# gregspangenberg/shoulder

Measured on AMD Instinct MI355X. Metric: humerus meshes/s end-to-end (all 4 landmarks), higher is better.
Workload: dtype f64 geometry + bf16 UNet

## Files before the change

shoulder_amd/csrc/hull.hip:

```cpp
#include "sh_ctx.h"

#include "k_hullpre.h"
#include "k_hull.h"
#include "sh_hull.h"

using namespace sh;

static int alloc_hulld(sh_ctx* c) {
  const int B = c->B;
  int rc;
  ENS("hulld.fv", (size_t)B * HD_SLOTS * 3 * 4, 4);
  ENS("hulld.vis", (size_t)B * HD_KC * HD_VMAX * 4, 4);
  ENS("hulld.ev", (size_t)B * HD_KC * 3 * HD_VMAX * 2 * 4, 4);
  ENS("hulld.hor", (size_t)B * HD_KC * (HD_VMAX + 2) * 2 * 4, 4);
  ENS("hulld.newslot", (size_t)B * HD_SLOTS * 4, 4);
  ENS("hulld.freestack", (size_t)B * HD_SLOTS * 4, 4);
  ENS("hulld.tkeys", (size_t)B * HD_TBL * 8, 8);
  ENS("hulld.tvals", (size_t)B * HD_TBL * 4, 4);
  ENS("hulld.fail", (size_t)B * 4, 4);
  ENS("hulld.rounds", (size_t)B * 4, 4);
  ENS("hulld.skip", (size_t)B * 4, 4);
  if (c->skip_gen != c->batch_gen) {
    HIPCHK(c, hipMemsetAsync(c->bufs["hulld.skip"].p, 0, (size_t)B * 4, c->stream));
    c->skip_gen = c->batch_gen;
    c->skip_nfmax = 0;
  }
  return SH_OK;
}

int sh::alloc_hullpre(sh_ctx* c, int B, long long sumV, const char* sfx) {
  const struct { const char* n; size_t per; int elem; } arr[] = {
      {"hullpre.ext", (size_t)SH_HP_NDIR * 4, 4}, {"hullpre.planes", (size_t)SH_HP_MAXPL * 4 * 8, 8}, {"hullpre.npl", 4, 4}, {"hullpre.nkept", 4, 4},
      {"hullpre.pval", (size_t)SH_HP_PARTS * SH_HP_NDIR * 8, 8}, {"hullpre.pidx", (size_t)SH_HP_PARTS * SH_HP_NDIR * 4, 4}, {"hullpre.pcnt", (size_t)SH_HP_PARTS * 4, 4},
      {"hullpre.poff", (size_t)SH_HP_PARTS * 8, 8}};
  const bool windows = sfx[0] == 0;
  int rc;
  for (const auto& a : arr) {
    const std::string nm = std::string(a.n) + sfx;
    if ((rc = ensure(c, nm.c_str(), (size_t)B * a.per, a.elem)) != SH_OK) return rc;
    c->bufs[nm].per_mesh = windows ? a.per : 0;
  }
  const std::string koff = std::string("hullpre.koff") + sfx, kept = std::string("hullpre.kept") + sfx;
  if ((rc = ensure(c, koff.c_str(), (size_t)(B + 1) * 8, 8)) != SH_OK) return rc;
  c->bufs[koff].per_mesh = windows ? (size_t)(B + 1) * 8 / (size_t)B : 0;
  if ((rc = ensure(c, kept.c_str(), (size_t)sumV * 12, 4)) != SH_OK) return rc;
  c->bufs[kept].per_mesh = windows ? (size_t)sumV * 12 / (size_t)B : 0;
  return SH_OK;
}

HullPre sh::hullpre_ptrs(sh_ctx* c, const char* sfx) {
  auto p = [&](const char* n) { return c->bufs[std::string(n) + sfx].p; };
  return HullPre{(const float*)p("verts"), (const long long*)p("voff"), (int*)p("hullpre.ext"), (double*)p("hullpre.planes"), (int*)p("hullpre.npl"), (float*)p("hullpre.kept"),
                 (int*)p("hullpre.nkept"), (long long*)p("hullpre.koff"), (double*)p("hullpre.pval"), (int*)p("hullpre.pidx"), (int*)p("hullpre.pcnt"), (long long*)p("hullpre.poff")};
}
static void launch_prefilter(const HullPre& hp, int B, hipStream_t st) {
  hipLaunchKernelGGL(k_hullpre_extremes, dim3(SH_HP_PARTS, B), dim3(256), 0, st, hp.verts, hp.voff, hp.pval, hp.pidx);
  hipLaunchKernelGGL(k_hullpre_polytope, dim3(B), dim3(256), 0, st, hp.verts, hp.voff, (const double*)hp.pval, (const int*)hp.pidx, hp.ext, hp.planes, hp.npl);
  hipLaunchKernelGGL(k_hullpre_filter<false>, dim3(SH_HP_PARTS, B), dim3(256), 0, st, hp.verts, hp.voff, (const double*)hp.planes, (const int*)hp.npl,
                     (const long long*)hp.poff, hp.kept, hp.pcnt);
  hipLaunchKernelGGL(k_hullpre_offsets, dim3(1), dim3(64), 0, st, (const int*)hp.pcnt, hp.koff, hp.poff, hp.nkept, B);
  hipLaunchKernelGGL(k_hullpre_filter<true>, dim3(SH_HP_PARTS, B), dim3(256), 0, st, hp.verts, hp.voff, (const double*)hp.planes, (const int*)hp.npl,
                     (const long long*)hp.poff, hp.kept, hp.pcnt);
}

hipError_t sh::fetch_prefiltered(const HullPre& hp, int B, long long sumV, long long* h_koff, float* h_kept, sh_ctx::HullPts* out, hipStream_t st) {
  hipError_t e;
  launch_prefilter(hp, B, st);
  if ((e = hipGetLastError()) != hipSuccess) return e;
  if ((e = hipMemcpyAsync(h_koff, hp.koff, (size_t)(B + 1) * 8, hipMemcpyDeviceToHost, st)) != hipSuccess) return e;
  if ((e = hipStreamSynchronize(st)) != hipSuccess) return e;
  const long long total = h_koff[B];
  if (total < 0 || total > sumV) return hipErrorUnknown;
  if (total > 0 && (e = hipMemcpyAsync(h_kept, hp.kept, (size_t)total * 12, hipMemcpyDeviceToHost, st)) != hipSuccess) return e;
  if ((e = hipStreamSynchronize(st)) != hipSuccess) return e;
  out->off.resize(B); out->cnt.resize(B);
  for (int b = 0; b < B; ++b) { out->off[b] = h_koff[b]; out->cnt[b] = (int)(h_koff[b + 1] - h_koff[b]); }
  out->src = h_kept;
  return hipSuccess;
}

hipError_t sh::fetch_hull_points(sh_ctx* c, const HullPre& hp, hipStream_t st) {
  const int B = c->B;
  sh_ctx::HullPts& in = c->hull_in;
  in.cnt.resize(B);
  if (c->h_verts_valid) {
    in.off.assign(c->h_voff.begin(), c->h_voff.begin() + B);
    for (int b = 0; b < B; ++b) in.cnt[b] = (int)(c->h_voff[b + 1] - c->h_voff[b]);
    in.src = c->h_verts.data();
    return hipSuccess;
  }
  hipError_t e;
  if (!c->sw.hull_prefilter || !hp.kept) {
    c->h_verts.resize(3 * (size_t)c->sumV);
    if ((e = hipMemcpyAsync(c->h_verts.data(), hp.verts, c->sumV * 3 * 4, hipMemcpyDeviceToHost, st)) != hipSuccess) return e;
    if ((e = hipStreamSynchronize(st)) != hipSuccess) return e;
    in.off.assign(c->h_voff.begin(), c->h_voff.begin() + B);
    for (int b = 0; b < B; ++b) in.cnt[b] = (int)(c->h_voff[b + 1] - c->h_voff[b]);
    in.src = c->h_verts.data();
    return hipSuccess;
  }
  return fetch_prefiltered(hp, B, c->sumV, c->h_koff, c->h_kept, &in, st);
}

class HullPool {
 public:
  static HullPool& instance() { static HullPool p; return p; }
  static unsigned thread_count() {
    unsigned nt = std::min(threads_per_local_rank(false), 32u);
    if (const char* e = getenv("SHOULDER_HULL_THREADS")) { int v = atoi(e); if (v > 0) nt = (unsigned)v; }
    return nt;
  }
  void run(const std::function<void()>& fn, int items) {
    Job job;
    job.fn = fn;
    job.want = (int)std::min<unsigned>(std::max(1, items), (unsigned)workers_.size() + 1) - 1;
    if (job.want > 0) {
      { std::lock_guard<std::mutex> lk(mu_); queue_.push_back(&job); }
      cv_.notify_all();
    }
    fn();
    if (job.want > 0) {
      std::unique_lock<std::mutex> lk(mu_);
      auto it = std::find(queue_.begin(), queue_.end(), &job);
      if (it != queue_.end()) queue_.erase(it);
      done_cv_.wait(lk, [&] { return job.active == 0; });
    }
  }

 private:
  struct Job { std::function<void()> fn; int want = 0, taken = 0, active = 0; };
  HullPool() {
    const unsigned nt = thread_count();
    for (unsigned t = 1; t < nt; ++t) workers_.emplace_back([this] { loop(); });
  }
  ~HullPool() {
    { std::lock_guard<std::mutex> lk(mu_); stop_ = true; }
    cv_.notify_all();
    for (auto& t : workers_) t.join();
  }
  void loop() {
    std::unique_lock<std::mutex> lk(mu_);
    for (;;) {
      cv_.wait(lk, [&] { return stop_ || !queue_.empty(); });
      if (stop_) return;
      Job* j = queue_.front();
      ++j->taken; ++j->active;
      if (j->taken >= j->want) queue_.pop_front();
      lk.unlock();
      j->fn();
      lk.lock();
      if (--j->active == 0) done_cv_.notify_all();
    }
  }
  std::mutex mu_;
  std::condition_variable cv_, done_cv_;
  std::deque<Job*> queue_;
  std::vector<std::thread> workers_;
  bool stop_ = false;
};

struct HullPhaseGate {
  std::mutex m; std::condition_variable cv; bool busy = false; std::atomic<int> fg_waiting{0};
  void enter(bool background) {
    std::unique_lock<std::mutex> l(m);
    if (!background) ++fg_waiting;
    cv.wait(l, [&] { return !busy && (!background || fg_waiting.load() == 0); });
    if (!background) --fg_waiting;
    busy = true;
  }
  bool foreground_waits() const { return fg_waiting.load(std::memory_order_relaxed) > 0; }
  void leave() { { std::lock_guard<std::mutex> l(m); busy = false; } cv.notify_all(); }
  static HullPhaseGate& instance() { static HullPhaseGate g; return g; }
};

int sh::hull_host_phase(sh_ctx* c, const sh_ctx::HullPts& in, int slot, int b0, int B, int* bad_mesh, double* ms, std::string* errtxt, bool background) {
  auto t0 = std::chrono::steady_clock::now();
  sh_ctx::HullStage& hs = c->hstage[slot];
  bool grown = false;
again:
  if (hs.cap < B || grown) {
    if (hs.hv) { (void)hipHostFree(hs.hv); (void)hipHostFree(hs.nr); (void)hipHostFree(hs.ed); (void)hipHostFree(hs.cnt); }
    hs.hv = nullptr; hs.cap = 0;
    HIPCHK_TXT(errtxt, hipHostMalloc((void**)&hs.hv, (size_t)B * hs.pv * 3 * 8));
    HIPCHK_TXT(errtxt, hipHostMalloc((void**)&hs.nr, (size_t)B * hs.pf * 3 * 8));
    HIPCHK_TXT(errtxt, hipHostMalloc((void**)&hs.ed, (size_t)B * hs.pe * 4 * 4));
    HIPCHK_TXT(errtxt, hipHostMalloc((void**)&hs.cnt, (size_t)B * 3 * 4));
    hs.cap = B;
  }
  if (!hs.ev) HIPCHK_TXT(errtxt, hipEventCreateWithFlags(&hs.ev, hipEventDisableTiming));
  if (hs.used) HIPCHK_TXT(errtxt, hipEventSynchronize(hs.ev));
  {
    sh_ctx::HullStage& ho = c->hstage[slot ^ 1];
    if (!ho.hv && !grown) {
      ho.pv = hs.pv; ho.pf = hs.pf; ho.pe = hs.pe;
      HIPCHK_TXT(errtxt, hipHostMalloc((void**)&ho.hv, (size_t)B * ho.pv * 3 * 8));
      HIPCHK_TXT(errtxt, hipHostMalloc((void**)&ho.nr, (size_t)B * ho.pf * 3 * 8));
      HIPCHK_TXT(errtxt, hipHostMalloc((void**)&ho.ed, (size_t)B * ho.pe * 4 * 4));
      HIPCHK_TXT(errtxt, hipHostMalloc((void**)&ho.cnt, (size_t)B * 3 * 4));
      ho.cap = B;
    }
  }
  double* hv = hs.hv; double* nr = hs.nr; int* ed = hs.ed; int* counts = hs.cnt;
  std::vector<int> status(B, 0);
  std::vector<int> demand(3 * (size_t)B, 0);
  std::atomic<int> next(0);
  auto work = [&]() {
    std::vector<double> P;
    shhull::Hull H;
    for (;;) {
      if (background && HullPhaseGate::instance().foreground_waits()) break;
      int b = next.fetch_add(1);
      if (b >= B) break;
      counts[b] = counts[B + b] = counts[2 * B + b] = 0;
      long long v0 = in.off[b0 + b], nv = in.cnt[b0 + b];
      P.resize(3 * (size_t)nv);
      const float* src = in.src + 3 * v0;
      for (long long i = 0; i < 3 * nv; ++i) P[i] = (double)src[i];
      if (!shhull::convex_hull(P.data(), (int)nv, H)) { status[b] = SH_ERR_GEOMETRY; continue; }
      int hn = (int)H.vert_ids.size(), fn = (int)H.tris.size() / 3, en = (int)H.edges.size() / 4;
      if (hn > hs.pv || fn > hs.pf || en > hs.pe) { status[b] = 1; demand[3 * (size_t)b] = hn; demand[3 * (size_t)b + 1] = fn; demand[3 * (size_t)b + 2] = en; continue; }
      for (int i = 0; i < hn; ++i)
        for (int k = 0; k < 3; ++k) hv[((size_t)b * hs.pv + i) * 3 + k] = P[3 * (size_t)H.vert_ids[i] + k];
      std::copy(H.normals.begin(), H.normals.end(), nr + (size_t)b * hs.pf * 3);
      std::copy(H.edges.begin(), H.edges.end(), ed + (size_t)b * hs.pe * 4);
      counts[b] = hn; counts[B + b] = fn; counts[2 * B + b] = en;
    }
  };
  do {
    HullPhaseGate::instance().enter(background);
    HullPool::instance().run(work, B);
    HullPhaseGate::instance().leave();
  } while (next.load() < B);
  if (!grown && std::find(status.begin(), status.end(), 1) != status.end()) {
    int dv = SH_HV, df = SH_HF, de = SH_HE;
    for (int b = 0; b < B; ++b) { dv = std::max(dv, demand[3 * (size_t)b]); df = std::max(df, demand[3 * (size_t)b + 1]); de = std::max(de, demand[3 * (size_t)b + 2]); }
    auto up = [](int x) { return (x + 1023) / 1024 * 1024; };
    hs.pv = up(dv); hs.pf = up(df); hs.pe = up(de);
    grown = true;
    std::fill(status.begin(), status.end(), 0);
    next = 0;
    goto again;
  }
  *ms = std::chrono::duration<double, std::milli>(std::chrono::steady_clock::now() - t0).count();
  for (int b = 0; b < B; ++b)
    if (status[b] != 0) { *bad_mesh = b0 + b; return status[b] == 1 ? SH_ERR_CAPACITY : status[b]; }
  return SH_OK;
}

hipError_t sh::hull_upload(sh_ctx* c, int slot, int B, const HullRec& dst, hipStream_t st) {
  sh_ctx::HullStage& hs = c->hstage[slot];
  const int* counts = hs.cnt;
  int nvmax = 1, nfmax = 1, nemax = 1;
  for (int b = 0; b < B; ++b) { nvmax = std::max(nvmax, counts[b]); nfmax = std::max(nfmax, counts[B + b]); nemax = std::max(nemax, counts[2 * B + b]); }
  if (nvmax > c->hcap.v || nfmax > c->hcap.f || nemax > c->hcap.e) return hipErrorInvalidValue;
  hipError_t e;
  if ((e = hipMemcpy2DAsync(dst.hv, (size_t)c->hcap.v * 24, hs.hv, (size_t)hs.pv * 24, (size_t)nvmax * 24, B, hipMemcpyHostToDevice, st)) != hipSuccess) return e;
  if ((e = hipMemcpy2DAsync(dst.normals, (size_t)c->hcap.f * 24, hs.nr, (size_t)hs.pf * 24, (size_t)nfmax * 24, B, hipMemcpyHostToDevice, st)) != hipSuccess) return e;
  if ((e = hipMemcpy2DAsync(dst.edges, (size_t)c->hcap.e * 16, hs.ed, (size_t)hs.pe * 16, (size_t)nemax * 16, B, hipMemcpyHostToDevice, st)) != hipSuccess) return e;
  if ((e = hipMemcpyAsync(dst.nv, counts, (size_t)B * 4, hipMemcpyHostToDevice, st)) != hipSuccess) return e;
  if ((e = hipMemcpyAsync(dst.nf, counts + B, (size_t)B * 4, hipMemcpyHostToDevice, st)) != hipSuccess) return e;
  if ((e = hipMemcpyAsync(dst.ne, counts + 2 * B, (size_t)B * 4, hipMemcpyHostToDevice, st)) != hipSuccess) return e;
  if ((e = hipEventRecord(hs.ev, st)) != hipSuccess) return e;
  hs.used = true;
  return hipSuccess;
}

int sh::run_device_hull(sh_ctx* c, int B, int* nfmax) {
  { int arc = alloc_hulld(c); if (arc != SH_OK) return arc; }
  launch_prefilter(hullpre_ptrs(c), B, c->stream);
  HIPCHK(c, hipGetLastError());
  HullScratch hs{buf<int>(c, "hulld.fv"), buf<int>(c, "hulld.vis"), buf<int>(c, "hulld.ev"), buf<int>(c, "hulld.hor"), buf<int>(c, "hulld.newslot"),
                 buf<int>(c, "hulld.freestack"), buf<unsigned long long>(c, "hulld.tkeys"), buf<unsigned>(c, "hulld.tvals")};
  const HullRec h = hull_rec(c);
  LAUNCH(c, "k_hull_rounds", k_hull_rounds, dim3(B), dim3(HD_THREADS), (const float*)c->bufs["hullpre.kept"].p, (const long long*)c->bufs["hullpre.koff"].p, hs,
         h.hv, h.normals, h.edges, h.nv, h.nf, h.ne,
         buf<int>(c, "hulld.fail"), buf<int>(c, "hulld.rounds"), (const int*)buf<int>(c, "hulld.skip"), c->hcap);
  LAUNCH(c, "k_hull_flag", k_hull_flag, dim3((B + 63) / 64), dim3(64), buf<int>(c, "hulld.fail"), buf<int>(c, "err"), B);
  *nfmax = std::max((int)HD_SLOTS, c->skip_nfmax);
  return SH_OK;
}
```

shoulder_amd/csrc/k_hullpre.h:

```cpp
#pragma once
#include "sh_common.h"

namespace sh {

#define SH_HP_NDIR 26
#define SH_HP_MAXPL 128
#define SH_HP_TOL 1e-6
#define SH_HP_MARGIN 1e-4

__device__ inline void hp_dir(int k, int* d) {
  const int t = k >= 13 ? k + 1 : k;
  d[0] = t % 3 - 1; d[1] = (t / 3) % 3 - 1; d[2] = t / 9 - 1;
}

#define SH_HP_PARTS 8

__global__ void __launch_bounds__(256)
k_hullpre_extremes(const float* __restrict__ verts, const long long* __restrict__ voff, double* __restrict__ pval ,
                   int* __restrict__ pidx ) {
  __shared__ double s_v[4][SH_HP_NDIR];
  __shared__ int s_i[4][SH_HP_NDIR];
  const int b = blockIdx.y, part = blockIdx.x, tid = threadIdx.x, lane = tid & 63, wave = tid >> 6;
  const long long v0 = voff[b];
  const int nv = (int)(voff[b + 1] - v0);
  const int per = (nv + SH_HP_PARTS - 1) / SH_HP_PARTS;
  const int a = min(nv, part * per), e = min(nv, a + per);
  const float* P = verts + 3 * v0;
  double best[SH_HP_NDIR];
  int bi[SH_HP_NDIR];
#pragma unroll
  for (int k = 0; k < SH_HP_NDIR; ++k) { best[k] = -1e300; bi[k] = 0x7fffffff; }
  for (int i = a + tid; i < e; i += 256) {
    const double x = P[3 * i], y = P[3 * i + 1], z = P[3 * i + 2];
#pragma unroll
    for (int k = 0; k < SH_HP_NDIR; ++k) {
      int d[3];
      hp_dir(k, d);
      const double v = (d[0] * x + d[1] * y) + d[2] * z;
      if (v > best[k]) { best[k] = v; bi[k] = i; }
    }
  }
#pragma unroll
  for (int k = 0; k < SH_HP_NDIR; ++k) {
    for (int off = 32; off > 0; off >>= 1) {
      const double ov = __shfl_down(best[k], off);
      const int oi = __shfl_down(bi[k], off);
      if (ov > best[k] || (ov == best[k] && oi < bi[k])) { best[k] = ov; bi[k] = oi; }
    }
    if (lane == 0) { s_v[wave][k] = best[k]; s_i[wave][k] = bi[k]; }
  }
  __syncthreads();
  if (tid < SH_HP_NDIR) {
    double v = s_v[0][tid];
    int i = s_i[0][tid];
    for (int w = 1; w < 4; ++w)
      if (s_v[w][tid] > v || (s_v[w][tid] == v && s_i[w][tid] < i)) { v = s_v[w][tid]; i = s_i[w][tid]; }
    pval[((size_t)b * SH_HP_PARTS + part) * SH_HP_NDIR + tid] = v;
    pidx[((size_t)b * SH_HP_PARTS + part) * SH_HP_NDIR + tid] = i;
  }
}

__global__ void __launch_bounds__(256)
k_hullpre_polytope(const float* __restrict__ verts, const long long* __restrict__ voff, const double* __restrict__ pval, const int* __restrict__ pidx,
                   int* __restrict__ ext , double* __restrict__ planes , int* __restrict__ nplanes ) {
  __shared__ double E[SH_HP_NDIR][3];
  __shared__ int id[SH_HP_NDIR];
  __shared__ int cnt;
  const int b = blockIdx.x, tid = threadIdx.x;
  if (tid < SH_HP_NDIR) {
    double v = -1e300;
    int i = 0x7fffffff;
    for (int part = 0; part < SH_HP_PARTS; ++part) {
      const double pv = pval[((size_t)b * SH_HP_PARTS + part) * SH_HP_NDIR + tid];
      const int pi = pidx[((size_t)b * SH_HP_PARTS + part) * SH_HP_NDIR + tid];
      if (pi != 0x7fffffff && (pv > v || (pv == v && pi < i))) { v = pv; i = pi; }
    }
    if (i == 0x7fffffff) i = -1;
    ext[b * SH_HP_NDIR + tid] = i;
    id[tid] = i;
    const float* p = verts + 3 * (voff[b] + (i < 0 ? 0 : i));
    E[tid][0] = p[0]; E[tid][1] = p[1]; E[tid][2] = p[2];
  }
  if (tid == 0) cnt = 0;
  __syncthreads();
  if (id[0] < 0) { if (tid == 0) nplanes[b] = -1; return; }
  constexpr int NT = SH_HP_NDIR * (SH_HP_NDIR - 1) * (SH_HP_NDIR - 2) / 6;
  double* PL = planes + (size_t)b * SH_HP_MAXPL * 4;
  for (int t = tid; t < NT; t += 256) {
    int i = 0, r = t;
    for (;; ++i) { const int c = (SH_HP_NDIR - 1 - i) * (SH_HP_NDIR - 2 - i) / 2; if (r < c) break; r -= c; }
    int j = i + 1;
    for (;; ++j) { const int c = SH_HP_NDIR - 1 - j; if (r < c) break; r -= c; }
    const int k = j + 1 + r;
    if (id[i] == id[j] || id[j] == id[k] || id[i] == id[k]) continue;
    const double ux = E[j][0] - E[i][0], uy = E[j][1] - E[i][1], uz = E[j][2] - E[i][2];
    const double vx = E[k][0] - E[i][0], vy = E[k][1] - E[i][1], vz = E[k][2] - E[i][2];
    double nx = uy * vz - uz * vy, ny = uz * vx - ux * vz, nz = ux * vy - uy * vx;
    const double nn = sqrt((nx * nx + ny * ny) + nz * nz);
    const double lu = sqrt((ux * ux + uy * uy) + uz * uz), lv = sqrt((vx * vx + vy * vy) + vz * vz);
    if (!(nn > 1e-9 * lu * lv)) continue;
    nx /= nn; ny /= nn; nz /= nn;
    const double d0 = (nx * E[i][0] + ny * E[i][1]) + nz * E[i][2];
    double smax = 0.0, smin = 0.0;
    for (int q = 0; q < SH_HP_NDIR; ++q) {
      const double s = ((nx * E[q][0] + ny * E[q][1]) + nz * E[q][2]) - d0;
      smax = fmax(smax, s); smin = fmin(smin, s);
    }
    double sg = 0.0;
    if (smax <= SH_HP_TOL && smin < -SH_HP_TOL) sg = 1.0;
    else if (smin >= -SH_HP_TOL && smax > SH_HP_TOL) sg = -1.0;
    if (sg == 0.0) continue;
    const int slot = atomicAdd(&cnt, 1);
    if (slot < SH_HP_MAXPL) { PL[4 * slot] = sg * nx; PL[4 * slot + 1] = sg * ny; PL[4 * slot + 2] = sg * nz; PL[4 * slot + 3] = sg * d0; }
  }
  __syncthreads();
  if (tid == 0) nplanes[b] = (cnt >= 4 && cnt <= SH_HP_MAXPL) ? cnt : -1;
}

__device__ inline bool hp_keep(const float* P, int i, const double* PL, int np) {
  if (np < 0) return true;
  const double x = P[3 * i], y = P[3 * i + 1], z = P[3 * i + 2];
  for (int q = 0; q < np; ++q)
    if (((PL[4 * q] * x + PL[4 * q + 1] * y) + PL[4 * q + 2] * z) - PL[4 * q + 3] >= -SH_HP_MARGIN) return true;
  return false;
}

template <bool WRITE>
__global__ void __launch_bounds__(256)
k_hullpre_filter(const float* __restrict__ verts, const long long* __restrict__ voff, const double* __restrict__ planes,
                 const int* __restrict__ nplanes, const long long* __restrict__ poff, float* __restrict__ kept, int* __restrict__ pcnt) {
  __shared__ double PL[SH_HP_MAXPL * 4];
  __shared__ int s_wave[2][4];
  const int b = blockIdx.y, part = blockIdx.x, tid = threadIdx.x, lane = tid & 63, wave = tid >> 6;
  const long long v0 = voff[b];
  const int nv = (int)(voff[b + 1] - v0);
  const int np = nplanes[b];
  for (int i = tid; i < 4 * max(np, 0); i += 256) PL[i] = planes[(size_t)b * SH_HP_MAXPL * 4 + i];
  __syncthreads();
  const float* P = verts + 3 * v0;
  const int per = (nv + SH_HP_PARTS - 1) / SH_HP_PARTS;
  const int a = min(nv, part * per), e = min(nv, a + per);
  float* K = WRITE ? kept + 3 * poff[(size_t)b * SH_HP_PARTS + part] : (float*)nullptr;
  int run = 0, it = 0;
  for (int base = a; base < e; base += 256, it ^= 1) {
    const int i = base + tid;
    const bool keep = i < e && hp_keep(P, i, PL, np);
    const unsigned long long bal = __ballot(keep);
    if (lane == 0) s_wave[it][wave] = __popcll(bal);
    __syncthreads();
    int woff = 0, total = 0;
#pragma unroll
    for (int w = 0; w < 4; ++w) { const int cw = s_wave[it][w]; if (w < wave) woff += cw; total += cw; }
    if (WRITE && keep) {
      const int pos = run + woff + __popcll(bal & (lane == 0 ? 0ull : (~0ull >> (64 - lane))));
      K[3 * pos] = P[3 * i]; K[3 * pos + 1] = P[3 * i + 1]; K[3 * pos + 2] = P[3 * i + 2];
    }
    run += total;
  }
  if (!WRITE && tid == 0) pcnt[(size_t)b * SH_HP_PARTS + part] = run;
}

__global__ void __launch_bounds__(64)
k_hullpre_offsets(const int* __restrict__ pcnt, long long* __restrict__ koff, long long* __restrict__ poff, int* __restrict__ nkept, int B) {
  const int lane = threadIdx.x;
  long long carry = 0;
  for (int base = 0; base < B; base += 64) {
    const int b = base + lane;
    int c[SH_HP_PARTS];
    long long mine = 0;
#pragma unroll
    for (int p = 0; p < SH_HP_PARTS; ++p) { c[p] = b < B ? pcnt[(size_t)b * SH_HP_PARTS + p] : 0; mine += c[p]; }
    long long incl = mine;
    for (int off = 1; off < 64; off <<= 1) { const long long t = __shfl_up(incl, off); if (lane >= off) incl += t; }
    long long acc = carry + incl - mine;
    if (b < B) {
      koff[b] = acc; nkept[b] = (int)mine;
#pragma unroll
      for (int p = 0; p < SH_HP_PARTS; ++p) { poff[(size_t)b * SH_HP_PARTS + p] = acc; acc += c[p]; }
    }
    carry += __shfl(incl, 63);
  }
  if (lane == 0) koff[B] = carry;
}

}
```

shoulder_amd/csrc/sh_ctx.h:

```cpp
#pragma once
#include "../../include/shoulder_hip.h"

#include <hip/hip_runtime.h>

#include <algorithm>
#include <atomic>
#include <chrono>
#include <cmath>
#include <condition_variable>
#include <cstddef>
#include <cstdio>
#include <cstring>
#include <deque>
#include <functional>
#include <initializer_list>
#include <map>
#include <memory>
#include <mutex>
#include <string>
#include <thread>
#include <tuple>
#include <vector>

#include "sh_arthro.h"
#include "sh_demand.h"
#include "sh_hullcap.h"
#include "sh_ingest.h"
#include "sh_unet_plan.h"

struct Buf {
  void* p = nullptr;
  size_t bytes = 0;
  int elem = 1;
  size_t per_mesh = 0;
};

struct KTimer {
  double ms = 0;
  int n = 0;
};

struct sh_ctx {
  int device = 0;
  hipStream_t stream = nullptr;
  bool own_stream = false;
  std::string err;
  sh_params params;
  int B = 0;
  long long sumV = 0, sumF = 0, maxV = 0, maxF = 0;
  std::vector<long long> h_voff, h_foff;
  std::map<std::string, Buf> bufs;
  bool have_rfc = false, have_unet = false;
  int rfc_nodes = 0, rfc_trees = 0;
  int unet_base = 0, unet_depth = 0;
  std::vector<float> h_unet;
  std::vector<int32_t> h_feat, h_ti, h_fi, h_roots;
  std::vector<float> h_thr, h_lw;
  typedef sh::UnetLayer ULayer;
  sh::UnetLayers ulayers;
  size_t unet_floats = 0;
  bool obb_injected = false;
  void* comm = nullptr;
  int comm_rank = -1, comm_n = 0;
  bool keep_products = false;
  int rs_cs_lo = 0, rs_cs_hi = 0;
  bool rs_all = false;
  unsigned long long rs_gen = ~0ull;
  int rec_rows = 0;
  int hull_mode = 1;
  unsigned long long skip_gen = ~0ull;
  int skip_nfmax = 0;
  unsigned long long ovf_seg_cap = 1ull << 18, ovf_ring_cap = 1ull << 18, ovf_work_cap = 32ull << 20;
  unsigned long long ovf_none_gen = ~0ull;
  int open_mode = SH_OPEN_ERROR;
  double open_gap = SH_OPEN_GAP_DEFAULT;
  int open_stats_run = SH_OPEN_ERROR;
  int end_cap = SH_ENDCAP;
  unsigned long long obb_gen = ~0ull;
  sh::HullCap hcap = {SH_HV, SH_HF, SH_HE};
  int obb_sil_need = 0;
  bool obb_nf_over = false;
  bool hull_force_host = false;
  std::vector<float> h_verts;
  bool h_verts_valid = false;
  float* h_kept = nullptr; long long h_kept_cap = 0;
  int* h_nkept = nullptr; int h_nkept_cap = 0;
  struct HullPts { const float* src = nullptr;
                   std::vector<long long> off;
                   std::vector<int> cnt; };
  HullPts hull_in;
  long long* h_koff = nullptr; int h_koff_cap = 0;
  struct StageSide {
    bool active = false, from_stl = false;
    int B = 0; long long sumV = 0, sumF = 0, maxV = 0, maxF = 0;
    std::vector<long long> voff, foff;
    void* h_src = nullptr; size_t h_src_cap = 0;
    int* h_flag = nullptr;
    size_t h_flag_cap = 0;
    float* h_kept = nullptr; long long h_kept_cap = 0;
    long long* h_koff = nullptr; int h_koff_cap = 0;
    HullPts pts;
    hipEvent_t ready_ev = nullptr;
    std::mutex m; std::condition_variable cv; bool meta_ready = true; int meta_rc = 0; std::string meta_err;
  } stg;
  int b0 = 0, Bwin = 0;
  struct HullStage { double* hv = nullptr; double* nr = nullptr; int* ed = nullptr; int* cnt = nullptr; int cap = 0; hipEvent_t ev = nullptr; bool used = false;
                     int pv = 4096, pf = 8192, pe = 12288; };
  HullStage hstage[2];
  int hslot = 0;
  struct Prepared {
    std::thread th; bool active = false; int slot = 0, B = 0, rc = SH_OK, bad_mesh = -1; unsigned long long gen = 0;
    double d2h_ms = 0, hull_ms = 0; std::string err;
    bool uploaded = false;
    bool staged = false;
  } prep;
  hipEvent_t obb_done_ev = nullptr;
  struct Ticket { hipEvent_t ev = nullptr; char* status = nullptr ; int cap = 0, B = 0; bool pending = false; sh_landmarks* host_out = nullptr;
                  uint32_t mask = 0; sh_landmarks* out_arg = nullptr; bool dev_hull = false; unsigned long long gen = 0; size_t rec = sizeof(sh_landmarks); int rows = 0; };
  Ticket tickets[2];
  int t_head = 0, t_tail = 0, n_pending = 0;
  hipStream_t out_stream = nullptr;
  bool overlap = false;
  unsigned long long batch_gen = 0;
  sh::ArthroState arthro;
  hipStream_t copy_stream = nullptr;
  hipEvent_t stl_counted_ev = nullptr;
  hipStream_t side_stream = nullptr;
  hipEvent_t side_fork_ev = nullptr, side_join_ev = nullptr;
  struct Switches {
    int window = 0;
    bool obb_prune = true;
    bool slice_merge = true;
    bool hull_prefilter = true;
    bool debug = false;
  } sw;
  struct Unet {
    bool reference = false;
    bool turn = false;
    hipEvent_t done_ev = nullptr;
    int num_cus = 0;
    int ticket_next = 0;
    std::map<std::tuple<int, int, int>, std::pair<int, int>> tk_tabs;
    int tk_tab_used = 0;
    bool zero_page_ready = false;
    bool packtab_ready = false;
    bool packed_x3 = false;
    int packed_kind = -1;
  } unet;
  bool packed_rfc = false;
  int timing = 0;
  std::vector<std::tuple<std::string, hipEvent_t, hipEvent_t>> pending;
  std::map<std::string, KTimer> timers;
};

#define HIPCHK(ctx, call)                                                                   \
  do {                                                                                      \
    hipError_t e_ = (call);                                                                 \
    if (e_ != hipSuccess) {                                                                 \
      (ctx)->err = std::string(#call) + ": " + hipGetErrorString(e_);                       \
      return SH_ERR_HIP;                                                                    \
    }                                                                                       \
  } while (0)

#define HIPCHK_TXT(errtxt, call) do { hipError_t e_ = (call); if (e_ != hipSuccess) { *(errtxt) = std::string(#call) + ": " + hipGetErrorString(e_); return SH_ERR_HIP; } } while (0)

struct WindowScope {
  sh_ctx* c; int b0, Bwin;
  WindowScope(sh_ctx* c_, int nb0, int nBwin) : c(c_), b0(c_->b0), Bwin(c_->Bwin) { c->b0 = nb0; c->Bwin = nBwin; }
  ~WindowScope() { c->b0 = b0; c->Bwin = Bwin; }
  WindowScope(const WindowScope&) = delete; WindowScope& operator=(const WindowScope&) = delete;
};

struct StreamScope {
  sh_ctx* c; hipStream_t saved;
  StreamScope(sh_ctx* c_, hipStream_t s) : c(c_), saved(c_->stream) { c->stream = s; }
  ~StreamScope() { c->stream = saved; }
  StreamScope(const StreamScope&) = delete; StreamScope& operator=(const StreamScope&) = delete;
};

static inline void params_changed(sh_ctx* c) { c->unet.packed_kind = -1; c->unet.packed_x3 = false; c->packed_rfc = false; }

static inline int fail(sh_ctx* c, int code, const std::string& msg) {
  if (c) c->err = msg;
  return code;
}

static inline int ensure(sh_ctx* c, const char* name, size_t bytes, int elem, void** out = nullptr) {
  Buf& b = c->bufs[name];
  if (b.bytes < bytes || b.p == nullptr) {
    if (b.p) (void)hipFree(b.p);
    b.p = nullptr;
    hipError_t e = hipMalloc(&b.p, bytes ? bytes : 16);
    if (e != hipSuccess) {
      c->err = std::string("hipMalloc(") + name + "): " + hipGetErrorString(e);
      b.bytes = 0;
      return SH_ERR_NOMEM;
    }
    b.bytes = bytes;
  }
  b.elem = elem;
  if (out) *out = b.p;
  return SH_OK;
}

template <typename T>
static inline T* buf(sh_ctx* c, const char* name) {
  auto it = c->bufs.find(name);
  if (it == c->bufs.end() || !it->second.p) return nullptr;
  return (T*)((char*)it->second.p + (size_t)c->b0 * it->second.per_mesh);
}

struct HullRec { double *hv, *normals; int *edges, *nv, *nf, *ne; };
static inline HullRec hull_rec(sh_ctx* c) {
  return {buf<double>(c, "hull.hv"), buf<double>(c, "hull.normals"), buf<int>(c, "hull.edges"), buf<int>(c, "hull.nv"), buf<int>(c, "hull.nf"), buf<int>(c, "hull.ne")};
}

#define ENS_(name, bytes, elem, per_mesh_)                                          \
  do {                                                                              \
    if ((rc = ensure(c, name, (size_t)(bytes), elem)) != SH_OK) return rc;          \
    c->bufs[name].per_mesh = (per_mesh_);                                           \
  } while (0)
#define ENS(name, bytes, elem) ENS_(name, bytes, elem, (size_t)(bytes) / (size_t)c->B)
#define ENS_SHARED(name, bytes, elem) ENS_(name, bytes, elem, 0)
template <typename T> constexpr int elem_of() { return sizeof(T) <= 8 ? (int)sizeof(T) : 1; }

static inline bool timed_launch(const sh_ctx* c, const char* name) {
  return c->timing == 1 || (c->timing == 2 && name[0] == 'u' && name[1] == 'n' && name[2] == 'e' && name[3] == 't' && name[4] == '.');
}

#define LAUNCH_FN(ctx, name, call)                                                           \
  do {                                                                                      \
    hipEvent_t e0_ = nullptr, e1_ = nullptr;                                                \
    const bool timed_ = timed_launch(ctx, name);                                            \
    if (timed_) {                                                                           \
      (void)hipEventCreate(&e0_); (void)hipEventCreate(&e1_);                               \
      (void)hipEventRecord(e0_, (ctx)->stream);                                             \
    }                                                                                       \
    call;                                                                                   \
    if (timed_) {                                                                           \
      (void)hipEventRecord(e1_, (ctx)->stream);                                             \
      (ctx)->pending.emplace_back(name, e0_, e1_);                                          \
    }                                                                                       \
    HIPCHK(ctx, hipGetLastError());                                                         \
  } while (0)
#define LAUNCH(ctx, name, kernel, grid, block, ...) LAUNCH_FN(ctx, name, hipLaunchKernelGGL(kernel, grid, block, 0, (ctx)->stream, __VA_ARGS__))

#define SH_REC_HEAD offsetof(sh_landmarks, anp_points)
#define SH_REC_TAIL (sizeof(sh_landmarks) - SH_REC_HEAD - sizeof(((sh_landmarks*)0)->anp_points))
static inline size_t rec_bytes_rows(int rows) { return rows > 0 ? SH_REC_HEAD + SH_REC_TAIL + (size_t)rows * 24 : sizeof(sh_landmarks); }

struct HullPre { const float* verts; const long long* voff; int* ext; double* planes; int* npl; float* kept; int* nkept; long long* koff; double* pval; int* pidx; int* pcnt; long long* poff; };
struct FillEnt { void* p; size_t bytes; unsigned char byte; };
struct UnetIO { const float* image; const double* raw; const unsigned long long* mm; float* logits; };
namespace sh {
int fill_list(sh_ctx* c, std::initializer_list<FillEnt> ents);
int emit_records(sh_ctx* c, void* dst, int b0, int n, int rows, size_t rec);
unsigned threads_per_local_rank(bool sustained = true);
HullPre hullpre_ptrs(sh_ctx* c, const char* sfx = "");
hipError_t fetch_prefiltered(const HullPre& hp, int B, long long sumV, long long* h_koff, float* h_kept, sh_ctx::HullPts* out, hipStream_t st);
hipError_t fetch_hull_points(sh_ctx* c, const HullPre& hp, hipStream_t st);
int hull_host_phase(sh_ctx* c, const sh_ctx::HullPts& in, int slot, int b0, int B, int* bad_mesh, double* ms, std::string* errtxt, bool background = false);
hipError_t hull_upload(sh_ctx* c, int slot, int B, const HullRec& dst, hipStream_t st);
int run_device_hull(sh_ctx* c, int B, int* nfmax);
int alloc_hullpre(sh_ctx* c, int B, long long sumV, const char* sfx);
int unet_turn_enter(sh_ctx* c);
int unet_turn_leave(sh_ctx* c);
void unet_turn_forget(sh_ctx* c);
int unet_dispatch(sh_ctx* c, const UnetIO& io, int nimg, int H, int W);
void comm_forget(sh_ctx* c);
}

#define FILL(ctx, ...) do { int frc_ = sh::fill_list(ctx, {__VA_ARGS__}); if (frc_ != SH_OK) return frc_; } while (0)
```

shoulder_amd/csrc/sh_hull.h:

```cpp
#pragma once
#include <algorithm>
#include <cmath>
#include <cstdint>
#include <vector>

namespace shhull {

struct Face {
  int v[3];
  int nb[3];
  double n[3], d;
  double area2 = 0.0;
  int head = -1;
  int far_pt = -1;
  double far_d = 0.0;
  bool alive = true;
  int mark = 0;
};

struct Hull {
  std::vector<int> vert_ids;
  std::vector<int> tris;
  std::vector<double> normals;
  std::vector<int> edges;
};

struct Builder {
  const double* P;
  int n;
  double eps;
  std::vector<Face> F;
  std::vector<int> next;

  double dist(const Face& f, int p) const { return f.n[0] * P[3 * p] + f.n[1] * P[3 * p + 1] + f.n[2] * P[3 * p + 2] - f.d; }

  void push(int f, int p, double d) {
    Face& fc = F[f];
    next[p] = fc.head;
    fc.head = p;
    if (fc.far_pt < 0 || d > fc.far_d) { fc.far_pt = p; fc.far_d = d; }
  }

  bool set_plane(Face& f) {
    const double* a = P + 3 * f.v[0]; const double* b = P + 3 * f.v[1]; const double* c = P + 3 * f.v[2];
    double u[3] = {b[0] - a[0], b[1] - a[1], b[2] - a[2]}, w[3] = {c[0] - a[0], c[1] - a[1], c[2] - a[2]};
    double nx = u[1] * w[2] - u[2] * w[1], ny = u[2] * w[0] - u[0] * w[2], nz = u[0] * w[1] - u[1] * w[0];
    double l = std::sqrt(nx * nx + ny * ny + nz * nz);
    f.area2 = l;
    if (l == 0.0) { f.n[0] = f.n[1] = 0; f.n[2] = 1; f.d = a[2]; return false; }
    f.n[0] = nx / l; f.n[1] = ny / l; f.n[2] = nz / l;
    f.d = f.n[0] * a[0] + f.n[1] * a[1] + f.n[2] * a[2];
    return true;
  }

  int add_face(int a, int b, int c) {
    Face f;
    f.v[0] = a; f.v[1] = b; f.v[2] = c;
    f.nb[0] = f.nb[1] = f.nb[2] = -1;
    set_plane(f);
    F.push_back(f);
    return (int)F.size() - 1;
  }
};

inline int& hull_fail_reason() { static thread_local int r = 0; return r; }
inline bool fail_(int why) { hull_fail_reason() = why; return false; }

inline bool convex_hull_eps(const double* pts_in, int n, Hull& H, double eps_rel) {
  if (n < 4) return fail_(1);
  std::vector<double> Pc(3 * (size_t)n);
  double c[3] = {0, 0, 0}, lo[3] = {1e300, 1e300, 1e300}, hi[3] = {-1e300, -1e300, -1e300};
  for (int i = 0; i < n; ++i)
    for (int k = 0; k < 3; ++k) { double v = pts_in[3 * i + k]; c[k] += v; lo[k] = std::min(lo[k], v); hi[k] = std::max(hi[k], v); }
  for (int k = 0; k < 3; ++k) c[k] /= n;
  for (int i = 0; i < n; ++i)
    for (int k = 0; k < 3; ++k) Pc[3 * (size_t)i + k] = pts_in[3 * i + k] - c[k];
  Builder B;
  B.P = Pc.data(); B.n = n;
  B.next.assign(n, -1);
  B.F.reserve(8192);
  double diag = std::sqrt((hi[0] - lo[0]) * (hi[0] - lo[0]) + (hi[1] - lo[1]) * (hi[1] - lo[1]) + (hi[2] - lo[2]) * (hi[2] - lo[2]));
  B.eps = eps_rel * diag;
  const double* P = B.P;
  int i0 = 0, i1 = 0;
  for (int i = 1; i < n; ++i) { if (P[3 * i] < P[3 * i0]) i0 = i; if (P[3 * i] > P[3 * i1]) i1 = i; }
  if (i0 == i1) return fail_(2);
  auto sub = [&](int a, int b, double* o) { for (int k = 0; k < 3; ++k) o[k] = P[3 * a + k] - P[3 * b + k]; };
  double e[3]; sub(i1, i0, e);
  int i2 = -1; double best = 0;
  for (int i = 0; i < n; ++i) {
    double w[3]; sub(i, i0, w);
    double cx = e[1] * w[2] - e[2] * w[1], cy = e[2] * w[0] - e[0] * w[2], cz = e[0] * w[1] - e[1] * w[0];
    double a2 = cx * cx + cy * cy + cz * cz;
    if (a2 > best) { best = a2; i2 = i; }
  }
  if (i2 < 0) return fail_(3);
  Face tmp; tmp.v[0] = i0; tmp.v[1] = i1; tmp.v[2] = i2; B.set_plane(tmp);
  int i3 = -1; best = 0;
  for (int i = 0; i < n; ++i) { double d = std::fabs(B.dist(tmp, i)); if (d > best) { best = d; i3 = i; } }
  if (i3 < 0 || best <= B.eps) return fail_(4);
  if (B.dist(tmp, i3) > 0) std::swap(i1, i2);
  int f0 = B.add_face(i0, i1, i2), f1 = B.add_face(i0, i3, i1), f2 = B.add_face(i1, i3, i2), f3 = B.add_face(i2, i3, i0);
  auto link = [&](int f, int ei, int g) { B.F[f].nb[ei] = g; };
  link(f0, 0, f1); link(f0, 1, f2); link(f0, 2, f3);
  link(f1, 0, f3); link(f1, 1, f2); link(f1, 2, f0);
  link(f2, 0, f1); link(f2, 1, f3); link(f2, 2, f0);
  link(f3, 0, f2); link(f3, 1, f1); link(f3, 2, f0);
  for (int p = 0; p < n; ++p) {
    if (p == i0 || p == i1 || p == i2 || p == i3) continue;
    for (int f = 0; f < 4; ++f) {
      double d = B.dist(B.F[f], p);
      if (d > B.eps) { B.push(f, p, d); break; }
    }
  }
  std::vector<int> stack, visible, horizon_f, horizon_e, pending, starts, ends, dropped, seen_start(n, 0), seen_end(n, 0);
  for (int f = 0; f < 4; ++f) if (B.F[f].head >= 0) pending.push_back(f);
  int stamp = 0, vstamp = 0;
  auto flood = [&](int f, int p, double thr) -> bool {
    ++stamp;
    visible.clear(); horizon_f.clear(); horizon_e.clear();
    stack.clear(); stack.push_back(f); B.F[f].mark = stamp;
    while (!stack.empty()) {
      int g = stack.back(); stack.pop_back();
      visible.push_back(g);
      for (int ei = 0; ei < 3; ++ei) {
        int h = B.F[g].nb[ei];
        if (h < 0 || h >= (int)B.F.size() || !B.F[h].alive) return fail_(5);
        if (B.F[h].mark == stamp) continue;
        if (B.dist(B.F[h], p) > thr) { B.F[h].mark = stamp; stack.push_back(h); }
        else { horizon_f.push_back(g); horizon_e.push_back(ei); }
      }
    }
    return true;
  };
  auto horizon_is_simple_loop = [&]() -> bool {
    const size_t m = horizon_f.size();
    if (m < 3) return fail_(6);
    ++vstamp;
    for (size_t k = 0; k < m; ++k) {
      const Face& g = B.F[horizon_f[k]];
      const int a = g.v[horizon_e[k]], b = g.v[(horizon_e[k] + 1) % 3];
      if (seen_start[a] == vstamp || seen_end[b] == vstamp) return fail_(7);
      seen_start[a] = vstamp; seen_end[b] = vstamp;
    }
    for (size_t k = 0; k < m; ++k) {
      const Face& g = B.F[horizon_f[k]];
      if (seen_start[g.v[(horizon_e[k] + 1) % 3]] != vstamp) return fail_(8);
    }
    std::vector<int>& nxt = stack;
    nxt.assign(m, -1);
    size_t steps = 0; int cur = 0;
    do {
      const Face& g = B.F[horizon_f[cur]];
      const int b = g.v[(horizon_e[cur] + 1) % 3];
      int found = -1;
      for (size_t k = 0; k < m; ++k) if (B.F[horizon_f[k]].v[horizon_e[k]] == b) { found = (int)k; break; }
      if (found < 0) return fail_(9);
      cur = found;
    } while (++steps < m && cur != 0);
    return cur == 0 && steps == m;
  };
  auto unlink_point = [&](int f, int p) {
    Face& fc = B.F[f];
    int prev = -1, q = fc.head;
    while (q >= 0 && q != p) { prev = q; q = B.next[q]; }
    if (q == p) { if (prev < 0) fc.head = B.next[p]; else B.next[prev] = B.next[p]; }
    fc.far_pt = -1; fc.far_d = 0.0;
    for (q = fc.head; q >= 0; q = B.next[q]) { const double d = B.dist(fc, q); if (fc.far_pt < 0 || d > fc.far_d) { fc.far_pt = q; fc.far_d = d; } }
  };
  for (int round = 0; round < 16; ++round) {
  if (round > 0) {
    std::vector<int> retry;
    retry.swap(dropped);
    bool any = false;
    for (int q : retry) {
      int bf = -1; double bd = B.eps;
      for (size_t fi = 0; fi < B.F.size(); ++fi)
        if (B.F[fi].alive) { const double d = B.dist(B.F[fi], q); if (d > bd) { bd = d; bf = (int)fi; } }
      if (bf >= 0) { B.push(bf, q, bd); pending.push_back(bf); any = true; }
    }
    if (!any) break;
  }
  while (!pending.empty()) {
    int f = pending.back(); pending.pop_back();
    if (!B.F[f].alive || B.F[f].head < 0) continue;
    const int p = B.F[f].far_pt;
    if (p < 0) return fail_(10);
    bool ok_h = flood(f, p, B.eps) && horizon_is_simple_loop();
    if (!ok_h) ok_h = flood(f, p, -100.0 * B.eps) && horizon_is_simple_loop();
    if (!ok_h) {
      unlink_point(f, p);
      dropped.push_back(p);
      if (B.F[f].head >= 0) pending.push_back(f);
      continue;
    }
    const size_t first_new = B.F.size();
    starts.clear(); ends.clear();
    for (size_t k = 0; k < horizon_f.size(); ++k) {
      int g = horizon_f[k], ei = horizon_e[k];
      int a = B.F[g].v[ei], b = B.F[g].v[(ei + 1) % 3];
      int h = B.F[g].nb[ei];
      int nf = B.add_face(a, b, p);
      starts.push_back(a); ends.push_back(b);
      B.F[nf].nb[0] = h;
      for (int q = 0; q < 3; ++q)
        if (B.F[h].nb[q] == g && B.F[h].v[q] == b && B.F[h].v[(q + 1) % 3] == a) B.F[h].nb[q] = nf;
    }
    const size_t nn = B.F.size() - first_new;
    for (size_t k = 0; k < nn; ++k) {
      int b = ends[k], a = starts[k];
      for (size_t m = 0; m < nn; ++m) {
        if (starts[m] == b) B.F[first_new + k].nb[1] = (int)(first_new + m);
        if (ends[m] == a) B.F[first_new + k].nb[2] = (int)(first_new + m);
      }
      if (B.F[first_new + k].nb[1] < 0 || B.F[first_new + k].nb[2] < 0) return fail_(11);
    }
    for (int g : visible) {
      int q = B.F[g].head;
      while (q >= 0) {
        int nx = B.next[q];
        if (q != p)
          for (size_t k = 0; k < nn; ++k) {
            double d = B.dist(B.F[first_new + k], q);
            if (d > B.eps) { B.push((int)(first_new + k), q, d); break; }
          }
        q = nx;
      }
      B.F[g].head = -1;
      B.F[g].alive = false;
    }
    for (size_t k = 0; k < nn; ++k) if (B.F[first_new + k].head >= 0) pending.push_back((int)(first_new + k));
  }
  if (dropped.empty()) break;
  }
  if (!dropped.empty()) {
    const double allow = std::max(100.0 * B.eps, 1e-6 * diag);
    for (int q : dropped)
      for (size_t fi = 0; fi < B.F.size(); ++fi)
        if (B.F[fi].alive && B.dist(B.F[fi], q) > allow) return fail_(12);
  }
  {
    const double allow = std::max(100.0 * B.eps, 1e-6 * diag);
    for (size_t fi = 0; fi < B.F.size(); ++fi) {
      if (!B.F[fi].alive) continue;
      const bool sliver = B.F[fi].area2 < 1e-7 * diag * diag;
      for (int k = 0; k < 3; ++k) {
        const int g = B.F[fi].nb[k];
        if (g < 0 || g >= (int)B.F.size() || !B.F[g].alive) return fail_(14);
        if (sliver) continue;
        for (int q = 0; q < 3; ++q) {
          const int w = B.F[g].v[q];
          if (w != B.F[fi].v[0] && w != B.F[fi].v[1] && w != B.F[fi].v[2] && B.dist(B.F[fi], w) > allow) return fail_(15);
        }
      }
    }
  }
  {
    double ctr[3];
    for (int k = 0; k < 3; ++k) ctr[k] = 0.25 * (P[3 * i0 + k] + P[3 * i1 + k] + P[3 * i2 + k] + P[3 * i3 + k]);
    for (size_t fi = 0; fi < B.F.size(); ++fi) {
      if (!B.F[fi].alive) continue;
      const double* a = P + 3 * B.F[fi].v[0]; const double* b = P + 3 * B.F[fi].v[1]; const double* c2 = P + 3 * B.F[fi].v[2];
      const double u[3] = {b[0] - a[0], b[1] - a[1], b[2] - a[2]}, w[3] = {c2[0] - a[0], c2[1] - a[1], c2[2] - a[2]};
      const double nx = u[1] * w[2] - u[2] * w[1], ny = u[2] * w[0] - u[0] * w[2], nz = u[0] * w[1] - u[1] * w[0];
      if (nx * (ctr[0] - a[0]) + ny * (ctr[1] - a[1]) + nz * (ctr[2] - a[2]) > 0.0) return fail_(16);
    }
  }
  std::vector<int> vmap(n, -1), fmap(B.F.size(), -1);
  H.vert_ids.clear(); H.tris.clear(); H.normals.clear(); H.edges.clear();
  int nf = 0;
  for (size_t f = 0; f < B.F.size(); ++f) {
    if (!B.F[f].alive) continue;
    fmap[f] = nf++;
    for (int k = 0; k < 3; ++k) {
      int v = B.F[f].v[k];
      if (vmap[v] < 0) { vmap[v] = (int)H.vert_ids.size(); H.vert_ids.push_back(v); }
      H.tris.push_back(vmap[v]);
    }
    {
      int r = 0;
      for (int k = 1; k < 3; ++k) if (B.F[f].v[k] < B.F[f].v[r]) r = k;
      double q[3][3];
      for (int k = 0; k < 3; ++k)
        for (int a = 0; a < 3; ++a) q[k][a] = pts_in[3 * (size_t)B.F[f].v[(r + k) % 3] + a] - 0.5 * (lo[a] + hi[a]);
      const double u[3] = {q[1][0] - q[0][0], q[1][1] - q[0][1], q[1][2] - q[0][2]}, w[3] = {q[2][0] - q[0][0], q[2][1] - q[0][1], q[2][2] - q[0][2]};
      const double nx = u[1] * w[2] - u[2] * w[1], ny = u[2] * w[0] - u[0] * w[2], nz = u[0] * w[1] - u[1] * w[0];
      const double l = std::sqrt(nx * nx + ny * ny + nz * nz);
      if (l == 0.0) { H.normals.push_back(0.0); H.normals.push_back(0.0); H.normals.push_back(1.0); }
      else { H.normals.push_back(nx / l); H.normals.push_back(ny / l); H.normals.push_back(nz / l); }
    }
  }
  for (size_t f = 0; f < B.F.size(); ++f) {
    if (!B.F[f].alive) continue;
    for (int k = 0; k < 3; ++k) {
      int g = B.F[f].nb[k];
      if (g < 0 || !B.F[g].alive) return fail_(13);
      if ((int)f < g) { H.edges.push_back(vmap[B.F[f].v[k]]); H.edges.push_back(vmap[B.F[f].v[(k + 1) % 3]]); H.edges.push_back(fmap[f]); H.edges.push_back(fmap[g]); }
    }
  }
  return true;
}

inline double joggle_unit(unsigned long long i, unsigned long long seed) {
  unsigned long long z = (i + 0x9E3779B97F4A7C15ull * (seed + 1));
  z = (z ^ (z >> 30)) * 0xBF58476D1CE4E5B9ull;
  z = (z ^ (z >> 27)) * 0x94D049BB133111EBull;
  z ^= z >> 31;
  return (double)(z >> 11) * (2.0 / 9007199254740992.0) - 1.0;
}

inline bool convex_hull(const double* pts_in, int n, Hull& H, int* how = nullptr) {
  if (convex_hull_eps(pts_in, n, H, 1e-10)) { if (how) *how = 0; return true; }
  if (n < 4) return false;
  double lo[3] = {1e300, 1e300, 1e300}, hi[3] = {-1e300, -1e300, -1e300};
  for (int i = 0; i < n; ++i)
    for (int k = 0; k < 3; ++k) { lo[k] = std::min(lo[k], pts_in[3 * i + k]); hi[k] = std::max(hi[k], pts_in[3 * i + k]); }
  const double diag = std::sqrt((hi[0] - lo[0]) * (hi[0] - lo[0]) + (hi[1] - lo[1]) * (hi[1] - lo[1]) + (hi[2] - lo[2]) * (hi[2] - lo[2]));
  std::vector<double> J(3 * (size_t)n);
  for (int attempt = 1; attempt <= 3; ++attempt) {
    const double amp = 1e-7 * diag * attempt;
    for (size_t i = 0; i < 3 * (size_t)n; ++i) J[i] = pts_in[i] + amp * joggle_unit(i, (unsigned long long)attempt);
    if (convex_hull_eps(J.data(), n, H, 1e-10)) {
      const size_t nf = H.tris.size() / 3;
      for (size_t f = 0; f < nf; ++f) {
        const double* a = pts_in + 3 * (size_t)H.vert_ids[H.tris[3 * f]]; const double* b = pts_in + 3 * (size_t)H.vert_ids[H.tris[3 * f + 1]];
        const double* c = pts_in + 3 * (size_t)H.vert_ids[H.tris[3 * f + 2]];
        const double u[3] = {b[0] - a[0], b[1] - a[1], b[2] - a[2]}, w[3] = {c[0] - a[0], c[1] - a[1], c[2] - a[2]};
        double nx = u[1] * w[2] - u[2] * w[1], ny = u[2] * w[0] - u[0] * w[2], nz = u[0] * w[1] - u[1] * w[0];
        const double l = std::sqrt(nx * nx + ny * ny + nz * nz);
        if (l > 0.0) { H.normals[3 * f] = nx / l; H.normals[3 * f + 1] = ny / l; H.normals[3 * f + 2] = nz / l; }
      }
      if (how) *how = attempt;
      return true;
    }
  }
  return false;
}

}
```

Baseline: 9188.

## Speed up hull prefilter kernels and CPU quickhull with reusable scratch and lookups

The GPU prefilter now computes 13 half-directions with paired max/min instead of 26 directional dots. The polytope kernel enumerates point pairs, uses a cheap 6-point pre-screen to queue candidate triples in a shared list, and runs the full face test only on queued triples. The filter's second pass reuses a per-vertex keep flag instead of recomputing plane tests. On the CPU side, quickhull reuses thread-local scratch buffers, splits cold face fields into a separate array, replaces linear horizon and neighbour searches with start/end index maps, and iterates a compacted live-face list. Together these cut kernel arithmetic and host allocation and search cost, at the price of more shared memory, an extra per-vertex buffer and considerably more complex code.

```diff
diff --git a/shoulder_amd/csrc/hull.hip b/shoulder_amd/csrc/hull.hip
--- a/shoulder_amd/csrc/hull.hip
+++ b/shoulder_amd/csrc/hull.hip
@@ -40,27 +40,29 @@
     if ((rc = ensure(c, nm.c_str(), (size_t)B * a.per, a.elem)) != SH_OK) return rc;
     c->bufs[nm].per_mesh = windows ? a.per : 0;
   }
-  const std::string koff = std::string("hullpre.koff") + sfx, kept = std::string("hullpre.kept") + sfx;
+  const std::string koff = std::string("hullpre.koff") + sfx, kept = std::string("hullpre.kept") + sfx, keep = std::string("hullpre.keep") + sfx;
   if ((rc = ensure(c, koff.c_str(), (size_t)(B + 1) * 8, 8)) != SH_OK) return rc;
   c->bufs[koff].per_mesh = windows ? (size_t)(B + 1) * 8 / (size_t)B : 0;
   if ((rc = ensure(c, kept.c_str(), (size_t)sumV * 12, 4)) != SH_OK) return rc;
   c->bufs[kept].per_mesh = windows ? (size_t)sumV * 12 / (size_t)B : 0;
+  if ((rc = ensure(c, keep.c_str(), (size_t)sumV, 1)) != SH_OK) return rc;
+  c->bufs[keep].per_mesh = 0;
   return SH_OK;
 }
 
 HullPre sh::hullpre_ptrs(sh_ctx* c, const char* sfx) {
   auto p = [&](const char* n) { return c->bufs[std::string(n) + sfx].p; };
   return HullPre{(const float*)p("verts"), (const long long*)p("voff"), (int*)p("hullpre.ext"), (double*)p("hullpre.planes"), (int*)p("hullpre.npl"), (float*)p("hullpre.kept"),
-                 (int*)p("hullpre.nkept"), (long long*)p("hullpre.koff"), (double*)p("hullpre.pval"), (int*)p("hullpre.pidx"), (int*)p("hullpre.pcnt"), (long long*)p("hullpre.poff")};
+                 (int*)p("hullpre.nkept"), (long long*)p("hullpre.koff"), (double*)p("hullpre.pval"), (int*)p("hullpre.pidx"), (int*)p("hullpre.pcnt"), (long long*)p("hullpre.poff"), (unsigned char*)p("hullpre.keep")};
 }
 static void launch_prefilter(const HullPre& hp, int B, hipStream_t st) {
   hipLaunchKernelGGL(k_hullpre_extremes, dim3(SH_HP_PARTS, B), dim3(256), 0, st, hp.verts, hp.voff, hp.pval, hp.pidx);
-  hipLaunchKernelGGL(k_hullpre_polytope, dim3(B), dim3(256), 0, st, hp.verts, hp.voff, (const double*)hp.pval, (const int*)hp.pidx, hp.ext, hp.planes, hp.npl);
+  hipLaunchKernelGGL(k_hullpre_polytope, dim3(B), dim3(SH_HP_PT), 0, st, hp.verts, hp.voff, (const double*)hp.pval, (const int*)hp.pidx, hp.ext, hp.planes, hp.npl);
   hipLaunchKernelGGL(k_hullpre_filter<false>, dim3(SH_HP_PARTS, B), dim3(256), 0, st, hp.verts, hp.voff, (const double*)hp.planes, (const int*)hp.npl,
-                     (const long long*)hp.poff, hp.kept, hp.pcnt);
+                     (const long long*)hp.poff, hp.kept, hp.pcnt, hp.keep);
   hipLaunchKernelGGL(k_hullpre_offsets, dim3(1), dim3(64), 0, st, (const int*)hp.pcnt, hp.koff, hp.poff, hp.nkept, B);
   hipLaunchKernelGGL(k_hullpre_filter<true>, dim3(SH_HP_PARTS, B), dim3(256), 0, st, hp.verts, hp.voff, (const double*)hp.planes, (const int*)hp.npl,
-                     (const long long*)hp.poff, hp.kept, hp.pcnt);
+                     (const long long*)hp.poff, hp.kept, hp.pcnt, hp.keep);
 }
 
 hipError_t sh::fetch_prefiltered(const HullPre& hp, int B, long long sumV, long long* h_koff, float* h_kept, sh_ctx::HullPts* out, hipStream_t st) {
@@ -205,8 +207,9 @@
   std::vector<int> demand(3 * (size_t)B, 0);
   std::atomic<int> next(0);
   auto work = [&]() {
-    std::vector<double> P;
-    shhull::Hull H;
+    static thread_local std::vector<double> P;
+    static thread_local shhull::Hull H;
+    static thread_local shhull::Scratch S;
     for (;;) {
       if (background && HullPhaseGate::instance().foreground_waits()) break;
       int b = next.fetch_add(1);
@@ -216,7 +219,7 @@
       P.resize(3 * (size_t)nv);
       const float* src = in.src + 3 * v0;
       for (long long i = 0; i < 3 * nv; ++i) P[i] = (double)src[i];
-      if (!shhull::convex_hull(P.data(), (int)nv, H)) { status[b] = SH_ERR_GEOMETRY; continue; }
+      if (!shhull::convex_hull(P.data(), (int)nv, H, nullptr, &S)) { status[b] = SH_ERR_GEOMETRY; continue; }
       int hn = (int)H.vert_ids.size(), fn = (int)H.tris.size() / 3, en = (int)H.edges.size() / 4;
       if (hn > hs.pv || fn > hs.pf || en > hs.pe) { status[b] = 1; demand[3 * (size_t)b] = hn; demand[3 * (size_t)b + 1] = fn; demand[3 * (size_t)b + 2] = en; continue; }
       for (int i = 0; i < hn; ++i)
diff --git a/shoulder_amd/csrc/k_hullpre.h b/shoulder_amd/csrc/k_hullpre.h
--- a/shoulder_amd/csrc/k_hullpre.h
+++ b/shoulder_amd/csrc/k_hullpre.h
@@ -3,14 +3,27 @@
 
 namespace sh {
 
-#define SH_HP_NDIR 26
+#define SH_HP_NHALF 13
+#define SH_HP_NDIR (2 * SH_HP_NHALF)
 #define SH_HP_MAXPL 128
+__device__ constexpr signed char HP_HALF[SH_HP_NHALF][3] = {
+    {1, 0, 0}, {0, 1, 0}, {0, 0, 1},
+    {1, 1, 0}, {1, -1, 0}, {1, 0, 1}, {1, 0, -1}, {0, 1, 1}, {0, 1, -1}, {1, 1, 1}, {1, 1, -1}, {1, -1, 1}, {1, -1, -1}};
 #define SH_HP_TOL 1e-6
 #define SH_HP_MARGIN 1e-4
 
-__device__ inline void hp_dir(int k, int* d) {
-  const int t = k >= 13 ? k + 1 : k;
-  d[0] = t % 3 - 1; d[1] = (t / 3) % 3 - 1; d[2] = t / 9 - 1;
+__device__ __forceinline__ double hp_dot(int h, const double* p , const double* p2 ) {
+  double v = 0.0;
+  bool first = true;
+#pragma unroll
+  for (int a = 0; a < 3; ++a) {
+    const int c = HP_HALF[h][a];
+    if (c == 0) continue;
+    const double t = (c == 2 || c == -2) ? p2[a] : p[a];
+    if (first) { v = c > 0 ? t : -t; first = false; }
+    else v = c > 0 ? v + t : v - t;
+  }
+  return v;
 }
 
 #define SH_HP_PARTS 8
@@ -26,28 +39,30 @@
   const int per = (nv + SH_HP_PARTS - 1) / SH_HP_PARTS;
   const int a = min(nv, part * per), e = min(nv, a + per);
   const float* P = verts + 3 * v0;
-  double best[SH_HP_NDIR];
-  int bi[SH_HP_NDIR];
-#pragma unroll
-  for (int k = 0; k < SH_HP_NDIR; ++k) { best[k] = -1e300; bi[k] = 0x7fffffff; }
+  double hi[SH_HP_NHALF], lo[SH_HP_NHALF];
+  int ihi[SH_HP_NHALF], ilo[SH_HP_NHALF];
+#pragma unroll
+  for (int h = 0; h < SH_HP_NHALF; ++h) { hi[h] = -1e300; lo[h] = 1e300; ihi[h] = ilo[h] = 0x7fffffff; }
   for (int i = a + tid; i < e; i += 256) {
-    const double x = P[3 * i], y = P[3 * i + 1], z = P[3 * i + 2];
-#pragma unroll
-    for (int k = 0; k < SH_HP_NDIR; ++k) {
-      int d[3];
-      hp_dir(k, d);
-      const double v = (d[0] * x + d[1] * y) + d[2] * z;
-      if (v > best[k]) { best[k] = v; bi[k] = i; }
+    const double p[3] = {(double)P[3 * i], (double)P[3 * i + 1], (double)P[3 * i + 2]};
+    const double p2[3] = {p[0] + p[0], p[1] + p[1], p[2] + p[2]};
+#pragma unroll
+    for (int h = 0; h < SH_HP_NHALF; ++h) {
+      const double v = hp_dot(h, p, p2);
+      if (v > hi[h]) { hi[h] = v; ihi[h] = i; }
+      if (v < lo[h]) { lo[h] = v; ilo[h] = i; }
     }
   }
 #pragma unroll
   for (int k = 0; k < SH_HP_NDIR; ++k) {
+    double bv = (k & 1) ? -lo[k >> 1] : hi[k >> 1];
+    int bi = (k & 1) ? ilo[k >> 1] : ihi[k >> 1];
     for (int off = 32; off > 0; off >>= 1) {
-      const double ov = __shfl_down(best[k], off);
-      const int oi = __shfl_down(bi[k], off);
-      if (ov > best[k] || (ov == best[k] && oi < bi[k])) { best[k] = ov; bi[k] = oi; }
-    }
-    if (lane == 0) { s_v[wave][k] = best[k]; s_i[wave][k] = bi[k]; }
+      const double ov = __shfl_down(bv, off);
+      const int oi = __shfl_down(bi, off);
+      if (ov > bv || (ov == bv && oi < bi)) { bv = ov; bi = oi; }
+    }
+    if (lane == 0) { s_v[wave][k] = bv; s_i[wave][k] = bi; }
   }
   __syncthreads();
   if (tid < SH_HP_NDIR) {
@@ -60,12 +75,39 @@
   }
 }
 
-__global__ void __launch_bounds__(256)
+__device__ inline void hp_try_face(const double (*E)[3], int i, int j, int k, double* __restrict__ PL, int* cnt) {
+  const double ox = E[i][0], oy = E[i][1], oz = E[i][2];
+  const double ux = E[j][0] - ox, uy = E[j][1] - oy, uz = E[j][2] - oz;
+  const double vx = E[k][0] - ox, vy = E[k][1] - oy, vz = E[k][2] - oz;
+  const double nx = uy * vz - uz * vy, ny = uz * vx - ux * vz, nz = ux * vy - uy * vx;
+  const double nn2 = (nx * nx + ny * ny) + nz * nz;
+  const double thr2 = (SH_HP_TOL * SH_HP_TOL) * nn2;
+  double smax = 0.0, smin = 0.0;
+  bool front = false, back = false;
+  for (int q = 0; q < SH_HP_NDIR; ++q) {
+    const double s = (nx * (E[q][0] - ox) + ny * (E[q][1] - oy)) + nz * (E[q][2] - oz);
+    smax = fmax(smax, s); smin = fmin(smin, s);
+    front = smax * smax > thr2; back = smin * smin > thr2;
+    if (front && back) return;
+  }
+  if (front == back) return;
+  const double sg = back ? 1.0 : -1.0;
+  const double nn = sqrt(nn2);
+  const double hx = nx / nn, hy = ny / nn, hz = nz / nn;
+  const double d0 = (hx * ox + hy * oy) + hz * oz;
+  const int slot = atomicAdd(cnt, 1);
+  if (slot < SH_HP_MAXPL) { PL[4 * slot] = sg * hx; PL[4 * slot + 1] = sg * hy; PL[4 * slot + 2] = sg * hz; PL[4 * slot + 3] = sg * d0; }
+}
+
+#define SH_HP_LIST 4096
+#define SH_HP_PT 512
+__global__ void __launch_bounds__(SH_HP_PT)
 k_hullpre_polytope(const float* __restrict__ verts, const long long* __restrict__ voff, const double* __restrict__ pval, const int* __restrict__ pidx,
                    int* __restrict__ ext , double* __restrict__ planes , int* __restrict__ nplanes ) {
   __shared__ double E[SH_HP_NDIR][3];
   __shared__ int id[SH_HP_NDIR];
-  __shared__ int cnt;
+  __shared__ unsigned list[SH_HP_LIST];
+  __shared__ int cnt, nlist;
   const int b = blockIdx.x, tid = threadIdx.x;
   if (tid < SH_HP_NDIR) {
     double v = -1e300;
@@ -81,39 +123,52 @@
     const float* p = verts + 3 * (voff[b] + (i < 0 ? 0 : i));
     E[tid][0] = p[0]; E[tid][1] = p[1]; E[tid][2] = p[2];
   }
-  if (tid == 0) cnt = 0;
+  if (tid == 0) { cnt = 0; nlist = 0; }
   __syncthreads();
   if (id[0] < 0) { if (tid == 0) nplanes[b] = -1; return; }
-  constexpr int NT = SH_HP_NDIR * (SH_HP_NDIR - 1) * (SH_HP_NDIR - 2) / 6;
+  constexpr int NP = SH_HP_NDIR * (SH_HP_NDIR - 1) / 2;
   double* PL = planes + (size_t)b * SH_HP_MAXPL * 4;
-  for (int t = tid; t < NT; t += 256) {
-    int i = 0, r = t;
-    for (;; ++i) { const int c = (SH_HP_NDIR - 1 - i) * (SH_HP_NDIR - 2 - i) / 2; if (r < c) break; r -= c; }
-    int j = i + 1;
-    for (;; ++j) { const int c = SH_HP_NDIR - 1 - j; if (r < c) break; r -= c; }
-    const int k = j + 1 + r;
-    if (id[i] == id[j] || id[j] == id[k] || id[i] == id[k]) continue;
-    const double ux = E[j][0] - E[i][0], uy = E[j][1] - E[i][1], uz = E[j][2] - E[i][2];
-    const double vx = E[k][0] - E[i][0], vy = E[k][1] - E[i][1], vz = E[k][2] - E[i][2];
-    double nx = uy * vz - uz * vy, ny = uz * vx - ux * vz, nz = ux * vy - uy * vx;
-    const double nn = sqrt((nx * nx + ny * ny) + nz * nz);
-    const double lu = sqrt((ux * ux + uy * uy) + uz * uz), lv = sqrt((vx * vx + vy * vy) + vz * vz);
-    if (!(nn > 1e-9 * lu * lv)) continue;
-    nx /= nn; ny /= nn; nz /= nn;
-    const double d0 = (nx * E[i][0] + ny * E[i][1]) + nz * E[i][2];
-    double smax = 0.0, smin = 0.0;
-    for (int q = 0; q < SH_HP_NDIR; ++q) {
-      const double s = ((nx * E[q][0] + ny * E[q][1]) + nz * E[q][2]) - d0;
-      smax = fmax(smax, s); smin = fmin(smin, s);
-    }
-    double sg = 0.0;
-    if (smax <= SH_HP_TOL && smin < -SH_HP_TOL) sg = 1.0;
-    else if (smin >= -SH_HP_TOL && smax > SH_HP_TOL) sg = -1.0;
-    if (sg == 0.0) continue;
-    const int slot = atomicAdd(&cnt, 1);
-    if (slot < SH_HP_MAXPL) { PL[4 * slot] = sg * nx; PL[4 * slot + 1] = sg * ny; PL[4 * slot + 2] = sg * nz; PL[4 * slot + 3] = sg * d0; }
-  }
-  __syncthreads();
+  for (int base = 0; base < NP; base += SH_HP_PT) {
+    const int t = base + tid;
+    if (t < NP) {
+      int i = 0, r = t;
+      for (;; ++i) { const int c = SH_HP_NDIR - 1 - i; if (r < c) break; r -= c; }
+      const int j = i + 1 + r;
+      if (id[i] != id[j]) {
+        const double ox = E[i][0], oy = E[i][1], oz = E[i][2];
+        const double ux = E[j][0] - ox, uy = E[j][1] - oy, uz = E[j][2] - oz;
+        const double lu2 = (ux * ux + uy * uy) + uz * uz;
+        for (int k = j + 1; k < SH_HP_NDIR; ++k) {
+          if (id[k] == id[i] || id[k] == id[j]) continue;
+          const double vx = E[k][0] - ox, vy = E[k][1] - oy, vz = E[k][2] - oz;
+          const double nx = uy * vz - uz * vy, ny = uz * vx - ux * vz, nz = ux * vy - uy * vx;
+          const double nn2 = (nx * nx + ny * ny) + nz * nz;
+          const double lv2 = (vx * vx + vy * vy) + vz * vz;
+          if (!(nn2 > 1e-18 * (lu2 * lv2))) continue;
+          const double thr2 = (SH_HP_TOL * SH_HP_TOL) * nn2;
+          double smax = 0.0, smin = 0.0;
+#pragma unroll
+          for (int q = 0; q < 6; ++q) {
+            const double s = (nx * (E[q][0] - ox) + ny * (E[q][1] - oy)) + nz * (E[q][2] - oz);
+            smax = fmax(smax, s); smin = fmin(smin, s);
+          }
+          if (smax * smax > thr2 && smin * smin > thr2) continue;
+          const int slot = atomicAdd(&nlist, 1);
+          if (slot < SH_HP_LIST) list[slot] = (unsigned)i | (unsigned)j << 8 | (unsigned)k << 16;
+          else hp_try_face(E, i, j, k, PL, &cnt);
+        }
+      }
+    }
+    __syncthreads();
+    const int n = min(nlist, SH_HP_LIST);
+    const bool last = base + SH_HP_PT >= NP;
+    if (last || n > SH_HP_LIST / 2) {
+      for (int e = tid; e < n; e += SH_HP_PT) { const unsigned w = list[e]; hp_try_face(E, (int)(w & 255u), (int)(w >> 8 & 255u), (int)(w >> 16), PL, &cnt); }
+      __syncthreads();
+      if (tid == 0) nlist = 0;
+    } else if (tid == 0) nlist = n;
+    __syncthreads();
+  }
   if (tid == 0) nplanes[b] = (cnt >= 4 && cnt <= SH_HP_MAXPL) ? cnt : -1;
 }
 
@@ -128,15 +183,18 @@
 template <bool WRITE>
 __global__ void __launch_bounds__(256)
 k_hullpre_filter(const float* __restrict__ verts, const long long* __restrict__ voff, const double* __restrict__ planes,
-                 const int* __restrict__ nplanes, const long long* __restrict__ poff, float* __restrict__ kept, int* __restrict__ pcnt) {
+                 const int* __restrict__ nplanes, const long long* __restrict__ poff, float* __restrict__ kept, int* __restrict__ pcnt,
+                 unsigned char* __restrict__ keepf ) {
   __shared__ double PL[SH_HP_MAXPL * 4];
   __shared__ int s_wave[2][4];
   const int b = blockIdx.y, part = blockIdx.x, tid = threadIdx.x, lane = tid & 63, wave = tid >> 6;
   const long long v0 = voff[b];
   const int nv = (int)(voff[b + 1] - v0);
-  const int np = nplanes[b];
-  for (int i = tid; i < 4 * max(np, 0); i += 256) PL[i] = planes[(size_t)b * SH_HP_MAXPL * 4 + i];
-  __syncthreads();
+  const int np = WRITE ? 0 : nplanes[b];
+  if (!WRITE) {
+    for (int i = tid; i < 4 * max(np, 0); i += 256) PL[i] = planes[(size_t)b * SH_HP_MAXPL * 4 + i];
+    __syncthreads();
+  }
   const float* P = verts + 3 * v0;
   const int per = (nv + SH_HP_PARTS - 1) / SH_HP_PARTS;
   const int a = min(nv, part * per), e = min(nv, a + per);
@@ -144,7 +202,8 @@
   int run = 0, it = 0;
   for (int base = a; base < e; base += 256, it ^= 1) {
     const int i = base + tid;
-    const bool keep = i < e && hp_keep(P, i, PL, np);
+    const bool keep = i < e && (WRITE ? keepf[v0 + i] != 0 : hp_keep(P, i, PL, np));
+    if (!WRITE && i < e) keepf[v0 + i] = keep ? 1 : 0;
     const unsigned long long bal = __ballot(keep);
     if (lane == 0) s_wave[it][wave] = __popcll(bal);
     __syncthreads();
diff --git a/shoulder_amd/csrc/sh_ctx.h b/shoulder_amd/csrc/sh_ctx.h
--- a/shoulder_amd/csrc/sh_ctx.h
+++ b/shoulder_amd/csrc/sh_ctx.h
@@ -249,7 +249,7 @@
 #define SH_REC_TAIL (sizeof(sh_landmarks) - SH_REC_HEAD - sizeof(((sh_landmarks*)0)->anp_points))
 static inline size_t rec_bytes_rows(int rows) { return rows > 0 ? SH_REC_HEAD + SH_REC_TAIL + (size_t)rows * 24 : sizeof(sh_landmarks); }
 
-struct HullPre { const float* verts; const long long* voff; int* ext; double* planes; int* npl; float* kept; int* nkept; long long* koff; double* pval; int* pidx; int* pcnt; long long* poff; };
+struct HullPre { const float* verts; const long long* voff; int* ext; double* planes; int* npl; float* kept; int* nkept; long long* koff; double* pval; int* pidx; int* pcnt; long long* poff; unsigned char* keep; };
 struct FillEnt { void* p; size_t bytes; unsigned char byte; };
 struct UnetIO { const float* image; const double* raw; const unsigned long long* mm; float* logits; };
 namespace sh {
diff --git a/shoulder_amd/csrc/sh_hull.h b/shoulder_amd/csrc/sh_hull.h
--- a/shoulder_amd/csrc/sh_hull.h
+++ b/shoulder_amd/csrc/sh_hull.h
@@ -10,12 +10,14 @@
   int v[3];
   int nb[3];
   double n[3], d;
+  int head = -1;
+  int mark = 0;
+  bool alive() const { return mark >= 0; }
+};
+struct FaceAux {
   double area2 = 0.0;
-  int head = -1;
+  double far_d = 0.0;
   int far_pt = -1;
-  double far_d = 0.0;
-  bool alive = true;
-  int mark = 0;
 };
 
 struct Hull {
@@ -25,28 +27,38 @@
   std::vector<int> edges;
 };
 
+struct Scratch {
+  std::vector<Face> F;
+  std::vector<FaceAux> A;
+  std::vector<double> Pc, J;
+  std::vector<int> next, stack, visible, horizon_f, horizon_e, pending, starts, ends, dropped, retry, seen_start, seen_end, start_at, end_at, vmap, fmap, live;
+};
+
 struct Builder {
   const double* P;
   int n;
   double eps;
-  std::vector<Face> F;
-  std::vector<int> next;
+  std::vector<Face>& F;
+  std::vector<FaceAux>& A;
+  std::vector<int>& next;
+  explicit Builder(Scratch& S) : F(S.F), A(S.A), next(S.next) {}
 
   double dist(const Face& f, int p) const { return f.n[0] * P[3 * p] + f.n[1] * P[3 * p + 1] + f.n[2] * P[3 * p + 2] - f.d; }
 
   void push(int f, int p, double d) {
     Face& fc = F[f];
+    FaceAux& fa = A[f];
     next[p] = fc.head;
     fc.head = p;
-    if (fc.far_pt < 0 || d > fc.far_d) { fc.far_pt = p; fc.far_d = d; }
-  }
-
-  bool set_plane(Face& f) {
+    if (fa.far_pt < 0 || d > fa.far_d) { fa.far_pt = p; fa.far_d = d; }
+  }
+
+  bool set_plane(Face& f, double* area2) {
     const double* a = P + 3 * f.v[0]; const double* b = P + 3 * f.v[1]; const double* c = P + 3 * f.v[2];
     double u[3] = {b[0] - a[0], b[1] - a[1], b[2] - a[2]}, w[3] = {c[0] - a[0], c[1] - a[1], c[2] - a[2]};
     double nx = u[1] * w[2] - u[2] * w[1], ny = u[2] * w[0] - u[0] * w[2], nz = u[0] * w[1] - u[1] * w[0];
     double l = std::sqrt(nx * nx + ny * ny + nz * nz);
-    f.area2 = l;
+    *area2 = l;
     if (l == 0.0) { f.n[0] = f.n[1] = 0; f.n[2] = 1; f.d = a[2]; return false; }
     f.n[0] = nx / l; f.n[1] = ny / l; f.n[2] = nz / l;
     f.d = f.n[0] * a[0] + f.n[1] * a[1] + f.n[2] * a[2];
@@ -54,11 +66,12 @@
   }
 
   int add_face(int a, int b, int c) {
-    Face f;
+    F.emplace_back();
+    A.emplace_back();
+    Face& f = F.back();
     f.v[0] = a; f.v[1] = b; f.v[2] = c;
     f.nb[0] = f.nb[1] = f.nb[2] = -1;
-    set_plane(f);
-    F.push_back(f);
+    set_plane(f, &A.back().area2);
     return (int)F.size() - 1;
   }
 };
@@ -66,19 +79,21 @@
 inline int& hull_fail_reason() { static thread_local int r = 0; return r; }
 inline bool fail_(int why) { hull_fail_reason() = why; return false; }
 
-inline bool convex_hull_eps(const double* pts_in, int n, Hull& H, double eps_rel) {
+inline bool convex_hull_eps(const double* pts_in, int n, Hull& H, double eps_rel, Scratch& S) {
   if (n < 4) return fail_(1);
-  std::vector<double> Pc(3 * (size_t)n);
+  std::vector<double>& Pc = S.Pc;
+  Pc.resize(3 * (size_t)n);
   double c[3] = {0, 0, 0}, lo[3] = {1e300, 1e300, 1e300}, hi[3] = {-1e300, -1e300, -1e300};
   for (int i = 0; i < n; ++i)
     for (int k = 0; k < 3; ++k) { double v = pts_in[3 * i + k]; c[k] += v; lo[k] = std::min(lo[k], v); hi[k] = std::max(hi[k], v); }
   for (int k = 0; k < 3; ++k) c[k] /= n;
   for (int i = 0; i < n; ++i)
     for (int k = 0; k < 3; ++k) Pc[3 * (size_t)i + k] = pts_in[3 * i + k] - c[k];
-  Builder B;
+  Builder B(S);
   B.P = Pc.data(); B.n = n;
   B.next.assign(n, -1);
-  B.F.reserve(8192);
+  B.F.clear(); B.A.clear();
+  B.F.reserve(16384); B.A.reserve(16384);
   double diag = std::sqrt((hi[0] - lo[0]) * (hi[0] - lo[0]) + (hi[1] - lo[1]) * (hi[1] - lo[1]) + (hi[2] - lo[2]) * (hi[2] - lo[2]));
   B.eps = eps_rel * diag;
   const double* P = B.P;
@@ -95,7 +110,7 @@
     if (a2 > best) { best = a2; i2 = i; }
   }
   if (i2 < 0) return fail_(3);
-  Face tmp; tmp.v[0] = i0; tmp.v[1] = i1; tmp.v[2] = i2; B.set_plane(tmp);
+  Face tmp; double tmp_area2; tmp.v[0] = i0; tmp.v[1] = i1; tmp.v[2] = i2; B.set_plane(tmp, &tmp_area2);
   int i3 = -1; best = 0;
   for (int i = 0; i < n; ++i) { double d = std::fabs(B.dist(tmp, i)); if (d > best) { best = d; i3 = i; } }
   if (i3 < 0 || best <= B.eps) return fail_(4);
@@ -113,7 +128,11 @@
       if (d > B.eps) { B.push(f, p, d); break; }
     }
   }
-  std::vector<int> stack, visible, horizon_f, horizon_e, pending, starts, ends, dropped, seen_start(n, 0), seen_end(n, 0);
+  std::vector<int>&stack = S.stack, &visible = S.visible, &horizon_f = S.horizon_f, &horizon_e = S.horizon_e, &pending = S.pending, &starts = S.starts, &ends = S.ends,
+                  &dropped = S.dropped, &retry = S.retry, &seen_start = S.seen_start, &seen_end = S.seen_end, &start_at = S.start_at, &end_at = S.end_at;
+  pending.clear(); dropped.clear();
+  seen_start.assign(n, 0); seen_end.assign(n, 0);
+  start_at.resize(n); end_at.resize(n);
   for (int f = 0; f < 4; ++f) if (B.F[f].head >= 0) pending.push_back(f);
   int stamp = 0, vstamp = 0;
   auto flood = [&](int f, int p, double thr) -> bool {
@@ -125,7 +144,7 @@
       visible.push_back(g);
       for (int ei = 0; ei < 3; ++ei) {
         int h = B.F[g].nb[ei];
-        if (h < 0 || h >= (int)B.F.size() || !B.F[h].alive) return fail_(5);
+        if (h < 0 || h >= (int)B.F.size() || !B.F[h].alive()) return fail_(5);
         if (B.F[h].mark == stamp) continue;
         if (B.dist(B.F[h], p) > thr) { B.F[h].mark = stamp; stack.push_back(h); }
         else { horizon_f.push_back(g); horizon_e.push_back(ei); }
@@ -142,49 +161,45 @@
       const int a = g.v[horizon_e[k]], b = g.v[(horizon_e[k] + 1) % 3];
       if (seen_start[a] == vstamp || seen_end[b] == vstamp) return fail_(7);
       seen_start[a] = vstamp; seen_end[b] = vstamp;
+      start_at[a] = (int)k; end_at[b] = (int)k;
     }
     for (size_t k = 0; k < m; ++k) {
       const Face& g = B.F[horizon_f[k]];
       if (seen_start[g.v[(horizon_e[k] + 1) % 3]] != vstamp) return fail_(8);
     }
-    std::vector<int>& nxt = stack;
-    nxt.assign(m, -1);
     size_t steps = 0; int cur = 0;
     do {
       const Face& g = B.F[horizon_f[cur]];
-      const int b = g.v[(horizon_e[cur] + 1) % 3];
-      int found = -1;
-      for (size_t k = 0; k < m; ++k) if (B.F[horizon_f[k]].v[horizon_e[k]] == b) { found = (int)k; break; }
-      if (found < 0) return fail_(9);
-      cur = found;
+      cur = start_at[g.v[(horizon_e[cur] + 1) % 3]];
     } while (++steps < m && cur != 0);
     return cur == 0 && steps == m;
   };
   auto unlink_point = [&](int f, int p) {
     Face& fc = B.F[f];
+    FaceAux& fa = B.A[f];
     int prev = -1, q = fc.head;
     while (q >= 0 && q != p) { prev = q; q = B.next[q]; }
     if (q == p) { if (prev < 0) fc.head = B.next[p]; else B.next[prev] = B.next[p]; }
-    fc.far_pt = -1; fc.far_d = 0.0;
-    for (q = fc.head; q >= 0; q = B.next[q]) { const double d = B.dist(fc, q); if (fc.far_pt < 0 || d > fc.far_d) { fc.far_pt = q; fc.far_d = d; } }
+    fa.far_pt = -1; fa.far_d = 0.0;
+    for (q = fc.head; q >= 0; q = B.next[q]) { const double d = B.dist(fc, q); if (fa.far_pt < 0 || d > fa.far_d) { fa.far_pt = q; fa.far_d = d; } }
   };
   for (int round = 0; round < 16; ++round) {
   if (round > 0) {
-    std::vector<int> retry;
+    retry.clear();
     retry.swap(dropped);
     bool any = false;
     for (int q : retry) {
       int bf = -1; double bd = B.eps;
       for (size_t fi = 0; fi < B.F.size(); ++fi)
-        if (B.F[fi].alive) { const double d = B.dist(B.F[fi], q); if (d > bd) { bd = d; bf = (int)fi; } }
+        if (B.F[fi].alive()) { const double d = B.dist(B.F[fi], q); if (d > bd) { bd = d; bf = (int)fi; } }
       if (bf >= 0) { B.push(bf, q, bd); pending.push_back(bf); any = true; }
     }
     if (!any) break;
   }
   while (!pending.empty()) {
     int f = pending.back(); pending.pop_back();
-    if (!B.F[f].alive || B.F[f].head < 0) continue;
-    const int p = B.F[f].far_pt;
+    if (!B.F[f].alive() || B.F[f].head < 0) continue;
+    const int p = B.A[f].far_pt;
     if (p < 0) return fail_(10);
     bool ok_h = flood(f, p, B.eps) && horizon_is_simple_loop();
     if (!ok_h) ok_h = flood(f, p, -100.0 * B.eps) && horizon_is_simple_loop();
@@ -208,12 +223,8 @@
     }
     const size_t nn = B.F.size() - first_new;
     for (size_t k = 0; k < nn; ++k) {
-      int b = ends[k], a = starts[k];
-      for (size_t m = 0; m < nn; ++m) {
-        if (starts[m] == b) B.F[first_new + k].nb[1] = (int)(first_new + m);
-        if (ends[m] == a) B.F[first_new + k].nb[2] = (int)(first_new + m);
-      }
-      if (B.F[first_new + k].nb[1] < 0 || B.F[first_new + k].nb[2] < 0) return fail_(11);
+      B.F[first_new + k].nb[1] = (int)first_new + start_at[ends[k]];
+      B.F[first_new + k].nb[2] = (int)first_new + end_at[starts[k]];
     }
     for (int g : visible) {
       int q = B.F[g].head;
@@ -227,26 +238,28 @@
         q = nx;
       }
       B.F[g].head = -1;
-      B.F[g].alive = false;
+      B.F[g].mark = -1;
     }
     for (size_t k = 0; k < nn; ++k) if (B.F[first_new + k].head >= 0) pending.push_back((int)(first_new + k));
   }
   if (dropped.empty()) break;
   }
+  std::vector<int>& live = S.live;
+  live.clear();
+  for (size_t fi = 0; fi < B.F.size(); ++fi) if (B.F[fi].alive()) live.push_back((int)fi);
   if (!dropped.empty()) {
     const double allow = std::max(100.0 * B.eps, 1e-6 * diag);
     for (int q : dropped)
-      for (size_t fi = 0; fi < B.F.size(); ++fi)
-        if (B.F[fi].alive && B.dist(B.F[fi], q) > allow) return fail_(12);
+      for (int fi : live)
+        if (B.dist(B.F[fi], q) > allow) return fail_(12);
   }
   {
     const double allow = std::max(100.0 * B.eps, 1e-6 * diag);
-    for (size_t fi = 0; fi < B.F.size(); ++fi) {
-      if (!B.F[fi].alive) continue;
-      const bool sliver = B.F[fi].area2 < 1e-7 * diag * diag;
+    for (int fi : live) {
+      const bool sliver = B.A[fi].area2 < 1e-7 * diag * diag;
       for (int k = 0; k < 3; ++k) {
         const int g = B.F[fi].nb[k];
-        if (g < 0 || g >= (int)B.F.size() || !B.F[g].alive) return fail_(14);
+        if (g < 0 || g >= (int)B.F.size() || !B.F[g].alive()) return fail_(14);
         if (sliver) continue;
         for (int q = 0; q < 3; ++q) {
           const int w = B.F[g].v[q];
@@ -258,19 +271,19 @@
   {
     double ctr[3];
     for (int k = 0; k < 3; ++k) ctr[k] = 0.25 * (P[3 * i0 + k] + P[3 * i1 + k] + P[3 * i2 + k] + P[3 * i3 + k]);
-    for (size_t fi = 0; fi < B.F.size(); ++fi) {
-      if (!B.F[fi].alive) continue;
+    for (int fi : live) {
       const double* a = P + 3 * B.F[fi].v[0]; const double* b = P + 3 * B.F[fi].v[1]; const double* c2 = P + 3 * B.F[fi].v[2];
       const double u[3] = {b[0] - a[0], b[1] - a[1], b[2] - a[2]}, w[3] = {c2[0] - a[0], c2[1] - a[1], c2[2] - a[2]};
       const double nx = u[1] * w[2] - u[2] * w[1], ny = u[2] * w[0] - u[0] * w[2], nz = u[0] * w[1] - u[1] * w[0];
       if (nx * (ctr[0] - a[0]) + ny * (ctr[1] - a[1]) + nz * (ctr[2] - a[2]) > 0.0) return fail_(16);
     }
   }
-  std::vector<int> vmap(n, -1), fmap(B.F.size(), -1);
+  std::vector<int>&vmap = S.vmap, &fmap = S.fmap;
+  vmap.assign(n, -1); fmap.assign(B.F.size(), -1);
   H.vert_ids.clear(); H.tris.clear(); H.normals.clear(); H.edges.clear();
+  H.tris.reserve(3 * live.size()); H.normals.reserve(3 * live.size()); H.edges.reserve(6 * live.size()); H.vert_ids.reserve(live.size() / 2 + 2);
   int nf = 0;
-  for (size_t f = 0; f < B.F.size(); ++f) {
-    if (!B.F[f].alive) continue;
+  for (int f : live) {
     fmap[f] = nf++;
     for (int k = 0; k < 3; ++k) {
       int v = B.F[f].v[k];
@@ -290,15 +303,19 @@
       else { H.normals.push_back(nx / l); H.normals.push_back(ny / l); H.normals.push_back(nz / l); }
     }
   }
-  for (size_t f = 0; f < B.F.size(); ++f) {
-    if (!B.F[f].alive) continue;
+  for (int f : live) {
     for (int k = 0; k < 3; ++k) {
       int g = B.F[f].nb[k];
-      if (g < 0 || !B.F[g].alive) return fail_(13);
-      if ((int)f < g) { H.edges.push_back(vmap[B.F[f].v[k]]); H.edges.push_back(vmap[B.F[f].v[(k + 1) % 3]]); H.edges.push_back(fmap[f]); H.edges.push_back(fmap[g]); }
+      if (g < 0 || !B.F[g].alive()) return fail_(13);
+      if (f < g) { H.edges.push_back(vmap[B.F[f].v[k]]); H.edges.push_back(vmap[B.F[f].v[(k + 1) % 3]]); H.edges.push_back(fmap[f]); H.edges.push_back(fmap[g]); }
     }
   }
   return true;
+}
+
+inline bool convex_hull_eps(const double* pts_in, int n, Hull& H, double eps_rel) {
+  Scratch S;
+  return convex_hull_eps(pts_in, n, H, eps_rel, S);
 }
 
 inline double joggle_unit(unsigned long long i, unsigned long long seed) {
@@ -309,18 +326,21 @@
   return (double)(z >> 11) * (2.0 / 9007199254740992.0) - 1.0;
 }
 
-inline bool convex_hull(const double* pts_in, int n, Hull& H, int* how = nullptr) {
-  if (convex_hull_eps(pts_in, n, H, 1e-10)) { if (how) *how = 0; return true; }
+inline bool convex_hull(const double* pts_in, int n, Hull& H, int* how = nullptr, Scratch* scratch = nullptr) {
+  Scratch own;
+  Scratch& S = scratch ? *scratch : own;
+  if (convex_hull_eps(pts_in, n, H, 1e-10, S)) { if (how) *how = 0; return true; }
   if (n < 4) return false;
   double lo[3] = {1e300, 1e300, 1e300}, hi[3] = {-1e300, -1e300, -1e300};
   for (int i = 0; i < n; ++i)
     for (int k = 0; k < 3; ++k) { lo[k] = std::min(lo[k], pts_in[3 * i + k]); hi[k] = std::max(hi[k], pts_in[3 * i + k]); }
   const double diag = std::sqrt((hi[0] - lo[0]) * (hi[0] - lo[0]) + (hi[1] - lo[1]) * (hi[1] - lo[1]) + (hi[2] - lo[2]) * (hi[2] - lo[2]));
-  std::vector<double> J(3 * (size_t)n);
+  std::vector<double>& J = S.J;
+  J.resize(3 * (size_t)n);
   for (int attempt = 1; attempt <= 3; ++attempt) {
     const double amp = 1e-7 * diag * attempt;
     for (size_t i = 0; i < 3 * (size_t)n; ++i) J[i] = pts_in[i] + amp * joggle_unit(i, (unsigned long long)attempt);
-    if (convex_hull_eps(J.data(), n, H, 1e-10)) {
+    if (convex_hull_eps(J.data(), n, H, 1e-10, S)) {
       const size_t nf = H.tris.size() / 3;
       for (size_t f = 0; f < nf; ++f) {
         const double* a = pts_in + 3 * (size_t)H.vert_ids[H.tris[3 * f]]; const double* b = pts_in + 3 * (size_t)H.vert_ids[H.tris[3 * f + 1]];
```

After: 9209, median of 5. Within noise of the previous version (+0.2%).
